# reidprichard/ORC

Measured on AMD Instinct MI355X. Metric: SIMPLE iterations/s (10.24M-cell hex channel equivalents; = iterations/s at N=1), higher is better.
Workload: dtype f64

## Files before the change

### include/orc_amd.h

```cpp
#ifndef ORC_AMD_H
#define ORC_AMD_H

#include <stdint.h>
#include "orc_types.h"

#ifdef __cplusplus
extern "C" {
#endif

typedef struct OrcMesh OrcMesh;
typedef struct OrcSolver OrcSolver;

int orc_init(int device_ordinal);
int orc_device_count(void);
int orc_synchronize(void);
const char *orc_status_string(int status);
const char *orc_last_error(void);
int orc_reload_environment(void);
int orc_device_memory(int64_t *free_bytes, int64_t *total_bytes);
int orc_device_info(char *buf, int cap);
void orc_settings_default(OrcSettings *s);

OrcMesh *orc_mesh_create(int64_t n_cells, int64_t n_faces, int32_t n_zones,
                         const int64_t *face_c0, const int64_t *face_c1, const int32_t *face_zone,
                         const double *face_area, const double *face_normal , const double *face_centroid ,
                         const double *cell_centroid , const double *cell_volume,
                         const int64_t *cell_face_ptr , const int64_t *cell_faces,
                         const int32_t *zone_type, const double *zone_scalar, const double *zone_vector ,
                         int *status);
OrcMesh *orc_mesh_create_reordered(int64_t n_cells, int64_t n_faces, int32_t n_zones,
                                   const int64_t *face_c0, const int64_t *face_c1, const int32_t *face_zone,
                                   const double *face_area, const double *face_normal, const double *face_centroid,
                                   const double *cell_centroid, const double *cell_volume,
                                   const int64_t *cell_face_ptr, const int64_t *cell_faces,
                                   const int32_t *zone_type, const double *zone_scalar, const double *zone_vector,
                                   int32_t ordering, int *status);
int orc_mesh_cell_order(const OrcMesh *m, int64_t *global_ids );
OrcMesh *orc_mesh_create_partitioned(int64_t n_owned, int64_t n_cells, int64_t n_cells_global, int64_t n_faces, int32_t n_zones,
                                     const int64_t *face_c0, const int64_t *face_c1, const int32_t *face_zone, const double *face_area,
                                     const double *face_normal, const double *face_centroid, const double *cell_centroid,
                                     const double *cell_volume, const int64_t *cell_face_ptr, const int64_t *cell_faces,
                                     const int32_t *zone_type, const double *zone_scalar, const double *zone_vector, int32_t n_peers,
                                     const int32_t *peers, const int64_t *send_ptr, const int64_t *send_idx, const int64_t *recv_ptr,
                                     int *status);
int64_t orc_mesh_n_owned(const OrcMesh *m);
typedef struct OrcPartition OrcPartition;
OrcPartition *orc_mesh_partition(int64_t n_cells, int64_t n_faces, const int64_t *face_c0, const int64_t *face_c1, const int32_t *face_zone,
                                 const double *face_area, const double *face_normal, const double *face_centroid,
                                 const double *cell_centroid, const double *cell_volume, const int64_t *cell_face_ptr,
                                 const int64_t *cell_faces, int32_t n_ranks, int32_t rank, int32_t ordering, int *status);
OrcPartition *orc_mesh_partition_owner(int64_t n_cells, int64_t n_faces, const int64_t *face_c0, const int64_t *face_c1, const int32_t *face_zone,
                                       const double *face_area, const double *face_normal, const double *face_centroid,
                                       const double *cell_centroid, const double *cell_volume, const int64_t *cell_face_ptr,
                                       const int64_t *cell_faces, const int32_t *cell_owner, int32_t n_ranks, int32_t rank, int64_t n_global,
                                       int *status);
void orc_partition_destroy(OrcPartition *p);
int orc_partition_sizes(const OrcPartition *p, int64_t *n_owned, int64_t *n_local, int64_t *n_global, int64_t *n_faces, int64_t *n_cell_faces,
                        int32_t *n_peers, int64_t *n_send);
int orc_partition_arrays(const OrcPartition *p, int64_t *face_c0, int64_t *face_c1, int32_t *face_zone, double *face_area, double *face_normal,
                         double *face_centroid, double *cell_centroid, double *cell_volume, int64_t *cell_face_ptr, int64_t *cell_faces,
                         int64_t *global_ids, int64_t *global_face_ids, int32_t *peers, int64_t *send_ptr, int64_t *send_idx, int64_t *recv_ptr);
OrcMesh *orc_partition_upload(const OrcPartition *p, int32_t n_zones, const int32_t *zone_type, const double *zone_scalar,
                              const double *zone_vector, int *status);
int orc_mesh_update_zones(OrcMesh *m, const int32_t *zone_type, const double *zone_scalar, const double *zone_vector);
void orc_mesh_destroy(OrcMesh *m);
int64_t orc_mesh_n_cells(const OrcMesh *m);
int64_t orc_mesh_nnz(const OrcMesh *m);
int orc_mesh_matrix_pattern(const OrcMesh *m, int64_t *row_ptr , int64_t *col_idx );

typedef struct OrcMeshData OrcMeshData;
OrcMeshData *orc_read_mesh(const char *mesh_path, int *status);
void orc_mesh_data_destroy(OrcMeshData *d);
int orc_mesh_data_sizes(const OrcMeshData *d, int32_t *dimensions, int64_t *n_vertices, int64_t *n_cells, int64_t *n_faces,
                        int64_t *n_cell_faces, int64_t *n_face_nodes, int32_t *n_zones);
int orc_mesh_data_arrays(const OrcMeshData *d, int64_t *face_c0, int64_t *face_c1, int32_t *face_zone, double *face_area,
                         double *face_normal, double *face_centroid, double *cell_centroid, double *cell_volume,
                         int64_t *cell_face_ptr, int64_t *cell_faces);
int orc_mesh_data_nodes(const OrcMeshData *d, double *vertices , int64_t *face_node_ptr , int64_t *face_nodes);
int orc_mesh_data_zone(const OrcMeshData *d, int32_t k, uint64_t *zone_id, int32_t *zone_type, double *scalar_value,
                       double *vector_value , char *name, int64_t name_len);
int orc_mesh_data_zone_index(const OrcMeshData *d, const char *name);
int orc_mesh_data_set_zone(OrcMeshData *d, const char *name, int32_t zone_type, double scalar_value, const double *vector_value );
OrcMesh *orc_mesh_upload(const OrcMeshData *d, int *status);
int orc_mesh_sync_zones(OrcMesh *m, const OrcMeshData *d);

int orc_write_data(const char *output_file_name, int64_t n_cells, const double *cell_centroid , const double *u,
                   const double *v, const double *w, const double *p, int decimal_precision);
int orc_read_data(const char *data_file_path, int64_t capacity, double *u, double *v, double *w, double *p, int64_t *n_read);
int orc_write_gradients(const OrcMesh *m, const double *cell_centroid, const double *u, const double *v, const double *w,
                        const double *p, const char *output_file_name, int decimal_precision, const OrcSettings *settings);

int orc_iterative_solve(int64_t n, const int64_t *row_ptr, const int64_t *col_idx, const double *values,
                        const double *b, double *solution_vector , uint64_t iteration_count,
                        int method , double relaxation_factor, double convergence_threshold,
                        int preconditioner );
int orc_iterative_solve3(int64_t n, const int64_t *row_ptr, const int64_t *col_idx, const double *const values[3],
                         const double *const b[3], double *const solution_vectors[3] , uint64_t iteration_count,
                         int method, double relaxation_factor, double convergence_threshold, int preconditioner,
                         int status_out[3]);
int orc_set_breakdown_guard(int on);
int64_t orc_breakdown_guard_events(int reset);
int orc_set_reduction_order(int order);
int64_t orc_last_jacobi_sweeps(void);
int orc_set_gmres_restart(int m);
int orc_last_gmres_stats(int64_t *steps, int64_t *cycles, double *initial_residual, double *final_estimate);
int orc_last_cg_stats(int64_t *iterations, double *initial_residual, double *final_residual, int32_t *event);
int orc_csr_spmv(int64_t n, const int64_t *row_ptr, const int64_t *col_idx, const double *values, const double *x,
                 double *y, int reps, double *avg_ms);

int orc_amg_coarsen(int64_t n, const int64_t *row_ptr, const int64_t *col_idx, const double *values, int64_t *partner ,
                    int64_t *out_n_coarse, int64_t *out_nnz, int64_t *out_row_ptr, int64_t *out_col, double *out_val,
                    int *rounds);

int orc_debug_coloring(int64_t n, const int64_t *row_ptr, const int64_t *col_idx, int32_t *colors , int32_t *n_colors);

int orc_build_momentum_diffusion_matrix(const OrcMesh *m, int diffusion_scheme, double mu,
                                        double *a_values , double *b_u, double *b_v, double *b_w);
int orc_initialize_momentum_matrix(const OrcMesh *m, double *a_values );
int orc_build_momentum_advection_matrices(const OrcMesh *m, double *a_u_values, double *a_v_values, double *a_w_values,
                                          double *b_u, double *b_v, double *b_w, const double *a_di_values,
                                          const double *u, const double *v, const double *w, const double *p,
                                          const OrcSettings *settings, double rho, double peclet[3]);
int orc_build_pressure_correction_matrices(const OrcMesh *m, const double *u, const double *v, const double *w,
                                           const double *p, const double *a_u_values, const double *a_v_values,
                                           const double *a_w_values, const OrcSettings *settings, double rho,
                                           double *a_values , double *b );

int orc_calculate_gradients(const OrcMesh *m, const double *u, const double *v, const double *w, const double *p,
                            const OrcSettings *settings, double *grad_p, double *grad_u);
int orc_check_boundary_conditions(const OrcMesh *m, int *constraint_type);
int orc_initialize_pressure_field(const OrcMesh *m, double *p );
int orc_initialize_flow(const OrcMesh *m, double mu, double rho, uint64_t iteration_count, const OrcSettings *settings,
                        double *u, double *v, double *w, double *p);
int orc_initialize_velocity_field(const OrcMesh *m, const OrcSettings *settings, double *u, double *v, double *w, double *psi);
int orc_initialize_flow_new(const OrcMesh *m, double mu, double rho, uint64_t iteration_count,
                            double *u, double *v, double *w, double *p);
typedef void (*OrcReportFn)(uint64_t iteration, const double mean_velocity[3], const double peclet[3],
                            double velocity_correction, double pressure_correction, double ms_per_iter, void *user);
int orc_solve_steady(OrcMesh *m, double *u, double *v, double *w, double *p, const OrcSettings *settings,
                     double rho, double mu, uint64_t iteration_count, uint64_t reporting_interval,
                     OrcReportFn report_cb, void *user);

OrcSolver *orc_solver_create(OrcMesh *m, const OrcSettings *settings, double rho, double mu, int *status);
void orc_solver_destroy(OrcSolver *s);
int orc_solver_set_fields(OrcSolver *s, const double *u, const double *v, const double *w, const double *p);
int orc_solver_get_fields(OrcSolver *s, double *u, double *v, double *w, double *p);
int orc_solver_iterate(OrcSolver *s, uint64_t iterations, double *report);
int orc_solver_snapshot(OrcSolver *s);
int orc_solver_restore(OrcSolver *s);
int orc_solver_set_pressure_solver(OrcSolver *s, const OrcLinearSolver *c);
int orc_solver_get_pressure_solver(OrcSolver *s, OrcLinearSolver *c, int32_t *enabled);
long long orc_solver_debug_pressure_hierarchies(OrcSolver *s);
int orc_solver_assemble_momentum(OrcSolver *s, double *a_u, double *a_v, double *a_w, double *b_u, double *b_v, double *b_w, double peclet[3]);
int orc_solver_assemble_pressure(OrcSolver *s, double *a_p, double *b_p);

int orc_solver_set_transient(OrcSolver *s, const OrcTransient *t);
int orc_solver_set_time_levels(OrcSolver *s, const double *u_n, const double *v_n, const double *w_n, const double *u_nm1,
                               const double *v_nm1, const double *w_nm1);
int orc_solver_advance(OrcSolver *s, uint64_t time_steps, double *report);
int orc_solve_transient(OrcMesh *m, double *u, double *v, double *w, double *p, const OrcSettings *settings, double rho, double mu,
                        const OrcTransient *t, uint64_t time_steps, uint64_t reporting_interval, OrcReportFn report_cb, void *user);

void orc_scalar_settings_default(OrcScalarSettings *c);
int orc_solver_set_scalar(OrcSolver *s, const OrcScalarSettings *c);
int orc_solver_set_scalar_bc(OrcSolver *s, int32_t zone, int32_t kind, double value);
int orc_solver_set_scalar_field(OrcSolver *s, const double *phi);
int orc_solver_get_scalar_field(OrcSolver *s, double *phi);
int orc_solver_set_scalar_source(OrcSolver *s, const double *source );
int orc_solver_set_scalar_levels(OrcSolver *s, const double *phi_n, const double *phi_nm1 );
int orc_solver_solve_scalar(OrcSolver *s, double report[4]);
int orc_solver_last_scalar_report(OrcSolver *s, double report[4]);
int orc_solver_assemble_scalar(OrcSolver *s, double *a, double *b);
int orc_solver_scalar_boundary_flux(OrcSolver *s, double *per_zone);

int orc_solver_surface_report(OrcSolver *s, const double origin[3], double *per_zone );
int orc_surface_integrals(OrcMesh *m, const double *u, const double *v, const double *w, const double *p,
                          double rho, double mu, const double origin[3], double *per_zone);
int orc_mesh_boundary_index(OrcMesh *m, int64_t *zone_ptr, int32_t *faces, int64_t *n_builds, int32_t *chunk);

int orc_solver_derived_fields(OrcSolver *s, uint32_t mask, double *out );
int orc_derived_fields(OrcMesh *m, const double *u, const double *v, const double *w, const OrcSettings *settings, uint32_t mask,
                       double *out);
int orc_solver_boundary_fields(OrcSolver *s, uint32_t mask, double *out );
int orc_boundary_fields(OrcMesh *m, const double *u, const double *v, const double *w, const double *p, double rho, double mu,
                        uint32_t mask, double *out);
int orc_write_vtu(const char *path, int64_t n_points, const double *points , int64_t n_cells, const int64_t *cell_face_ptr,
                  const int64_t *cell_faces, const int64_t *face_node_ptr, const int64_t *face_nodes, int32_t n_arrays,
                  const char *const *names, const int32_t *components, const double *const *data, int32_t encoding);
int orc_write_vtu_faces(const char *path, int64_t n_points, const double *points, int64_t n_faces, const int64_t *face_ids,
                        const int64_t *face_node_ptr, const int64_t *face_nodes, int32_t n_arrays, const char *const *names,
                        const int32_t *components, const double *const *data, int32_t encoding);

int orc_bench_spmv(OrcSolver *s, int reps, double *avg_ms, double *checksum);
int orc_bench_bicgstab_iteration(OrcSolver *s, int reps, double *avg_ms);
int orc_bench_inloop_products(OrcSolver *s, int reps, double avg_ms[4]);
const char *orc_bench_inloop_variant(void);
int orc_bench_gs_sweep(OrcSolver *s, int reps, double *avg_ms, int *n_colors);
int orc_bench_gs_sweep0(OrcSolver *s, int reps, double avg_ms[2], int *n_colors);
int orc_bench_amg_levels(OrcSolver *s, int reps, int64_t *rows, int64_t *nnz, int64_t *padded, double *avg_ms, int *n_levels);
long long orc_debug_halo_overlaps(void);
int orc_debug_stream_report(char *buf, int cap);
int orc_debug_amg_coarse_product(int64_t n, const int64_t *row_ptr, const int64_t *col_idx, const double *values, int scaled, const double *x,
                                 double *y, int *has_window_mirror);
int orc_debug_amg_packed_mirror(int64_t n, const int64_t *row_ptr, const int64_t *col_idx, const double *values, int64_t sizes[5], int32_t *row_len,
                                int64_t *pk_ptr, int32_t *pk_col, double *pk_val, int64_t *lptr, uint16_t *lidx, int32_t *wcol, int32_t *wsize);
long long orc_debug_collectives(int reset);
int orc_debug_clamp_partials_grid(long long requested);
int orc_debug_max_partials(void);
int orc_debug_amg_certification(long long out[2], int reset);
int orc_debug_amg_setup_stats(long long out[16], int reset);
int orc_debug_xwin_counters(long long out[3], int reset);
long long orc_debug_shared_galerkin(int reset);
enum {
    ORC_PRODUCT_RAGGED = 0,
    ORC_PRODUCT_PACKED = 1,
    ORC_PRODUCT_WINDOW = 2,
    ORC_PRODUCT_GENERIC_SCALED = 3,
    ORC_PRODUCT_WIDE = 4,
    ORC_PRODUCT_NARROW = 5,
    ORC_PRODUCT_NARROW_NT = 6,
    ORC_PRODUCT_MESH = 7,
    ORC_PRODUCT_FAMILIES = 8
};
int orc_debug_product_launches(long long *out, int n_out, int reset);
int orc_profile_enable(int on);
int orc_profile_report(char *buf, int64_t buf_len);

int orc_hex_channel_sizes(int64_t nx, int64_t ny, int64_t nz, int64_t *n_cells, int64_t *n_faces, int64_t *n_cell_faces);
int orc_hex_channel_generate(int64_t nx, int64_t ny, int64_t nz, double lx, double ly, double lz,
                             int64_t *face_c0, int64_t *face_c1, int32_t *face_zone, double *face_area,
                             double *face_normal, double *face_centroid, double *cell_centroid, double *cell_volume,
                             int64_t *cell_face_ptr, int64_t *cell_faces);
int orc_hex_channel_write_msh(const char *path, int64_t nx, int64_t ny, int64_t nz, double lx, double ly, double lz);

int orc_mixed_channel_write_msh(const char *path, int64_t nx, int64_t ny, int64_t nz, double lx, double ly, double lz,
                                int64_t *n_cells, int64_t *n_faces);
int orc_poly_channel_write_msh(const char *path, int64_t nx, int64_t ny, int64_t nz, double lx, double ly, double lz,
                               int64_t *n_cells, int64_t *n_faces);
OrcMeshData *orc_mixed_channel_generate(int64_t nx, int64_t ny, int64_t nz, double lx, double ly, double lz, int polyhedra, int *status);

#define ORC_COMM_ID_BYTES 128
int orc_comm_get_unique_id(unsigned char id[ORC_COMM_ID_BYTES]);
int orc_comm_init(const unsigned char id[ORC_COMM_ID_BYTES], int rank, int world_size);
int orc_comm_finalize(void);
int orc_comm_selftest(void);
int orc_comm_init_self_loop(void);
int orc_comm_set_host_transport(void *exchange_fn, void *allreduce_fn, void *user);

#ifdef __cplusplus
}
#endif
#endif
```

### orc_amd/csrc/amg_hooks.hip

```cpp
#include <algorithm>

#include "amg.hpp"

namespace orc {

static int build_level(const MatView &A, Arena &arena, AmgHierarchy::Level &L) {
    const int64_t n = A.P.n;
    ORC_TRY(arena.alloc((size_t)std::max<int64_t>(n, 1), &L.choice));
    ORC_TRY(arena.alloc((size_t)std::max<int64_t>(n, 1), &L.chooser));
    ORC_TRY(aggregate(A, arena, L.choice, L.chooser, &L.rounds));
    return galerkin(A, arena, L);
}

int amg_debug_coarsen(const MatView &A, Arena &arena, std::vector<int> &choice_h, std::vector<int64_t> &row_ptr_h,
                      std::vector<int64_t> &col_h, std::vector<double> &val_h, int *rounds, const double *x_h, double *y_h, int scaled, int *mirror_out) {
    const int64_t n = A.P.n;
    hipStream_t st = ctx().stream;
    ArenaScope scope(arena);
    AmgHierarchy::Level L;
    ORC_TRY(build_level(A, arena, L));
    if (rounds) *rounds = L.rounds;
    choice_h.resize((size_t)n);
    ORC_HIP(hipMemcpyAsync(choice_h.data(), L.choice, sizeof(int) * (size_t)n, hipMemcpyDeviceToHost, st));
    const int64_t nc = L.n;
    if (mirror_out) *mirror_out = (L.pk.ptr && L.xw.lidx) ? 1 : 0;
    if (x_h && y_h && nc > 0) {
        MatView V = coarse_view(L, A.symmetric);
        double *x, *y, *d1;
        ORC_TRY(arena.alloc((size_t)nc, &x));
        ORC_TRY(arena.alloc((size_t)nc, &y));
        ORC_HIP(hipMemcpyAsync(x, x_h, sizeof(double) * (size_t)nc, hipMemcpyHostToDevice, st));
        if (scaled) {
            ORC_TRY(arena.alloc((size_t)nc, &d1));
            ORC_TRY(diag_inverse_dev(V, d1));
            V.s1 = d1;
            ORC_TRY(materialize_scaled_view(V, 50, arena));
        }
        ORC_TRY(spmv_dev(V, x, y));
        ORC_HIP(hipMemcpyAsync(y_h, y, sizeof(double) * (size_t)nc, hipMemcpyDeviceToHost, st));
        ORC_HIP(hipStreamSynchronize(st));
    }
    std::vector<int> row_len((size_t)nc), col((size_t)std::max<int64_t>(L.padded, 1));
    std::vector<int64_t> slice_ptr((size_t)L.P.n_slices + 1);
    std::vector<double> val((size_t)std::max<int64_t>(L.padded, 1));
    ORC_HIP(hipMemcpyAsync(row_len.data(), L.P.row_len, sizeof(int) * (size_t)nc, hipMemcpyDeviceToHost, st));
    ORC_HIP(hipMemcpyAsync(slice_ptr.data(), L.P.slice_ptr, sizeof(int64_t) * slice_ptr.size(), hipMemcpyDeviceToHost, st));
    ORC_HIP(hipMemcpyAsync(col.data(), L.P.col, sizeof(int) * (size_t)L.padded, hipMemcpyDeviceToHost, st));
    ORC_HIP(hipMemcpyAsync(val.data(), L.val, sizeof(double) * (size_t)L.padded, hipMemcpyDeviceToHost, st));
    ORC_HIP(hipStreamSynchronize(st));
    row_ptr_h.assign((size_t)nc + 1, 0);
    for (int64_t I = 0; I < nc; ++I) row_ptr_h[(size_t)I + 1] = row_ptr_h[(size_t)I] + row_len[(size_t)I];
    col_h.resize((size_t)row_ptr_h[(size_t)nc]);
    val_h.resize((size_t)row_ptr_h[(size_t)nc]);
    for (int64_t I = 0; I < nc; ++I) {
        const int64_t base = slice_ptr[(size_t)(I >> 6)] + (I & 63);
        for (int k = 0; k < row_len[(size_t)I]; ++k) {
            col_h[(size_t)(row_ptr_h[(size_t)I] + k)] = col[(size_t)(base + (int64_t)k * 64)];
            val_h[(size_t)(row_ptr_h[(size_t)I] + k)] = val[(size_t)(base + (int64_t)k * 64)];
        }
    }
    return ORC_OK;
}

int amg_debug_packed(const MatView &A, Arena &arena, int64_t sizes[5], int32_t *row_len_h, int64_t *pk_ptr_h, int32_t *pk_col_h, double *pk_val_h,
                     int64_t *lptr_h, uint16_t *lidx_h, int32_t *wcol_h, int32_t *wsize_h) {
    hipStream_t st = ctx().stream;
    ArenaScope scope(arena);
    AmgHierarchy::Level L;
    ORC_TRY(build_level(A, arena, L));
    const bool mirror = L.pk.ptr && L.xw.lidx;
    const int64_t ns = L.P.n_slices, nb = (ns + 3) / 4;
    sizes[0] = L.n; sizes[1] = ns; sizes[2] = mirror ? L.pk.slots : 0; sizes[3] = 0; sizes[4] = mirror ? nb : 0;
    if (mirror) ORC_HIP(hipMemcpyAsync(&sizes[3], L.xw.lptr + ns, sizeof(int64_t), hipMemcpyDeviceToHost, st));
    ORC_HIP(hipStreamSynchronize(st));
    if (mirror && row_len_h && pk_ptr_h && pk_col_h && pk_val_h && lptr_h && lidx_h && wcol_h && wsize_h) {
        ORC_HIP(hipMemcpyAsync(row_len_h, L.P.row_len, sizeof(int32_t) * (size_t)L.n, hipMemcpyDeviceToHost, st));
        ORC_HIP(hipMemcpyAsync(pk_ptr_h, L.pk.ptr, sizeof(int64_t) * (size_t)(ns + 1), hipMemcpyDeviceToHost, st));
        ORC_HIP(hipMemcpyAsync(pk_col_h, L.pk.col, sizeof(int32_t) * (size_t)sizes[2], hipMemcpyDeviceToHost, st));
        ORC_HIP(hipMemcpyAsync(pk_val_h, L.pk.val, sizeof(double) * (size_t)sizes[2], hipMemcpyDeviceToHost, st));
        ORC_HIP(hipMemcpyAsync(lptr_h, L.xw.lptr, sizeof(int64_t) * (size_t)(ns + 1), hipMemcpyDeviceToHost, st));
        ORC_HIP(hipMemcpyAsync(lidx_h, L.xw.lidx, sizeof(uint16_t) * (size_t)sizes[3], hipMemcpyDeviceToHost, st));
        ORC_HIP(hipMemcpyAsync(wcol_h, L.xw.wcol, sizeof(int32_t) * (size_t)(nb * kXWinCap), hipMemcpyDeviceToHost, st));
        ORC_HIP(hipMemcpyAsync(wsize_h, L.xw.wsize, sizeof(int32_t) * (size_t)nb, hipMemcpyDeviceToHost, st));
        ORC_HIP(hipStreamSynchronize(st));
    }
    return ORC_OK;
}

}
```

### orc_amd/csrc/amg_mirror.hip

```cpp
#include <algorithm>

#include "amg.hpp"

namespace orc {

constexpr int kXBitWords = 8192;
__device__ unsigned long long g_xwin_counters[3];
constexpr int kXBitWordsSmall = 4096;
template <int kWords, bool kSecond>
__global__ __launch_bounds__(kBlock) void xwin_build_k(SellDev P, const int64_t *__restrict__ lptr, int *__restrict__ wcol, int *__restrict__ wsize,
                                                       unsigned short *__restrict__ lidx, int64_t n_blocks, int win_cap, int bit_words, int pass_words,
                                                       int *__restrict__ pending ) {
    if (kSecond && *pending == 0) return;
    __shared__ unsigned bits[kWords];
    __shared__ unsigned short wpre[kWords];
    __shared__ int s_min, s_max, s_part[kBlock];
    const int tid = threadIdx.x, lane = tid & 63, wave = tid >> 6;
    unsigned long long n_built = 0, n_capped = 0, n_spanned = 0;
    for (int64_t b = blockIdx.x; b < n_blocks; b += gridDim.x) {
        if (kSecond && wsize[b] != -2) continue;
        const int64_t row = b * kXWinRows + tid;
        const bool live = row < P.n;
        const int len = live ? P.row_len[row] : 0;
        const int64_t rbase = live ? P.slice_ptr[row >> 6] + (row & 63) : 0;
        if (tid == 0) { s_min = 0x7fffffff; s_max = -1; }
        __syncthreads();
        if (len > 0) {
            atomicMin(&s_min, P.col[rbase]);
            atomicMax(&s_max, P.col[rbase + (int64_t)(len - 1) * 64]);
        }
        __syncthreads();
        const int cmin = s_min, span = s_max - s_min + 1;
        const int words = (span + 31) >> 5;
        if (s_max < 0) {
            if (tid == 0) wsize[b] = 0;
            __syncthreads();
            continue;
        }
        if (!kSecond && words <= bit_words && words > pass_words) {
            if (tid == 0) { wsize[b] = -2; atomicAdd(pending, 1); }
            __syncthreads();
            continue;
        }
        ++n_built;
        if (words > bit_words || words > kWords) {
            if (tid == 0) wsize[b] = -1;
            ++n_spanned;
            __syncthreads();
            continue;
        }
        for (int w = tid; w < words; w += kBlock) bits[w] = 0u;
        __syncthreads();
        for (int k = 0; k < len; ++k) {
            const int c = P.col[rbase + (int64_t)k * 64] - cmin;
            atomicOr(&bits[c >> 5], 1u << (c & 31));
        }
        __syncthreads();
        const int per = (words + kBlock - 1) / kBlock;
        int local = 0;
        for (int w = tid * per; w < words && w < (tid + 1) * per; ++w) local += __popc(bits[w]);
        s_part[tid] = local;
        __syncthreads();
        for (int off = 1; off < kBlock; off <<= 1) {
            const int t = tid >= off ? s_part[tid - off] : 0;
            __syncthreads();
            s_part[tid] += t;
            __syncthreads();
        }
        const int total = s_part[kBlock - 1];
        if (total > win_cap) {
            __syncthreads();
            if (tid == 0) wsize[b] = -1;
            ++n_capped;
            __syncthreads();
            continue;
        }
        int run = s_part[tid] - local;
        int *wc = wcol + b * kXWinCap;
        for (int w = tid * per; w < words && w < (tid + 1) * per; ++w) {
            wpre[w] = (unsigned short)run;
            unsigned m = bits[w];
            while (m) {
                const int bit = __ffs(m) - 1;
                wc[run++] = cmin + (w << 5) + bit;
                m &= m - 1;
            }
        }
        if (tid == 0) wsize[b] = total;
        __syncthreads();
        const int64_t slice = b * 4 + wave;
        if (slice < P.n_slices) {
            const int64_t sbase = P.slice_ptr[slice];
            const int width = (int)((P.slice_ptr[slice + 1] - sbase) >> 6);
            int64_t off = lptr[slice];
            for (int j0 = 0; j0 < width; j0 += kPackChunk) {
                const bool in = j0 < len;
                const unsigned long long m = __ballot(in);
                const int rank = __builtin_amdgcn_mbcnt_hi((unsigned)(m >> 32), __builtin_amdgcn_mbcnt_lo((unsigned)m, 0u));
                if (in) {
                    u32x4_t w = {0u, 0u, 0u, 0u};
#pragma unroll
                    for (int u = 0; u < kPackChunk; ++u) {
                        if (j0 + u < len) {
                            const int c = P.col[sbase + (int64_t)(j0 + u) * 64 + lane] - cmin;
                            const unsigned pos = wpre[c >> 5] + __popc(bits[c >> 5] & ((1u << (c & 31)) - 1u));
                            w[u >> 1] |= pos << (16 * (u & 1));
                        }
                    }
                    *reinterpret_cast<u32x4_t *>(lidx + off + (int64_t)kPackChunk * rank) = w;
                }
                off += (int64_t)kPackChunk * __popcll(m);
            }
        }
        __syncthreads();
    }
    if (tid == 0) {
        if (n_built) atomicAdd(&g_xwin_counters[0], n_built);
        if (n_capped) atomicAdd(&g_xwin_counters[1], n_capped);
        if (n_spanned) atomicAdd(&g_xwin_counters[2], n_spanned);
    }
}

constexpr int kXWinCapSizes = 5;
__device__ __constant__ int kXWinCapSizeDev[kXWinCapSizes] = {2048, 2560, 3200, 4000, kXWinCap};
static const int kXWinCapSize[kXWinCapSizes] = {2048, 2560, 3200, 4000, kXWinCap};
__global__ __launch_bounds__(kBlock) void xwin_cap_k(const int *__restrict__ wsize, int64_t n_blocks, int *__restrict__ over) {
    int c[kXWinCapSizes] = {0, 0, 0, 0, 0};
    for (int64_t b = (int64_t)blockIdx.x * blockDim.x + threadIdx.x; b < n_blocks; b += (int64_t)gridDim.x * blockDim.x) {
        const int ws = wsize[b];
#pragma unroll
        for (int q = 0; q < kXWinCapSizes; ++q) c[q] += ws > kXWinCapSizeDev[q] ? 1 : 0;
    }
#pragma unroll
    for (int q = 0; q < kXWinCapSizes; ++q)
        if (c[q]) atomicAdd(over + q, c[q]);
}

__global__ __launch_bounds__(kBlock) void xwin_stats_k(const int *__restrict__ wcol, const int *__restrict__ wsize, int64_t n_blocks, unsigned long long *__restrict__ out) {
    for (int64_t b = blockIdx.x; b < n_blocks; b += gridDim.x) {
        const int ws = wsize[b];
        if (ws <= 0) { if (threadIdx.x == 0 && ws < 0) atomicAdd(out + 4, 1ull); continue; }
        const int *wc = wcol + b * kXWinCap;
        unsigned long long runs = 0, long_entries = 0;
        for (int j = threadIdx.x; j < ws; j += kBlock) {
            if (j == 0 || wc[j] != wc[j - 1] + 1) {
                ++runs;
                int e = j + 1;
                while (e < ws && wc[e] == wc[e - 1] + 1) ++e;
                if (e - j >= 8) long_entries += (unsigned long long)(e - j);
            }
        }
        atomicAdd(out + 1, runs);
        atomicAdd(out + 2, long_entries);
        if (threadIdx.x == 0) {
            atomicAdd(out + 0, (unsigned long long)ws);
            if (wc[ws - 1] - wc[0] < 65536) atomicAdd(out + 3, 1ull);
        }
    }
}

__global__ __launch_bounds__(64) void narrow_build_k(SellDev P, unsigned short *__restrict__ col16, int *__restrict__ colbase, int *__restrict__ too_wide) {
    const int lane = threadIdx.x;
    for (int64_t slice = blockIdx.x; slice < P.n_slices; slice += gridDim.x) {
        const int64_t row = slice * 64 + lane;
        const int64_t sb = P.slice_ptr[slice];
        const int width = (int)((P.slice_ptr[slice + 1] - sb) >> 6);
        const int len = row < P.n ? P.row_len[row] : 0;
        for (int k = 0; k < width; ++k) {
            const bool in = k < len;
            const int c = in ? P.col[sb + (int64_t)k * 64 + lane] : 0;
            int lo = in ? c : 0x7fffffff, hi = in ? c : -1;
#pragma unroll
            for (int off = 32; off > 0; off >>= 1) {
                lo = min(lo, __shfl_xor(lo, off, 64));
                hi = max(hi, __shfl_xor(hi, off, 64));
            }
            if (hi < 0) lo = 0;
            if (lane == 0) {
                colbase[(sb >> 6) + k] = lo;
                if (hi >= 0 && hi - lo > 65535) atomicOr(too_wide, 1);
            }
            col16[sb + (int64_t)k * 64 + lane] = in ? (unsigned short)(c - lo) : (unsigned short)0;
        }
    }
}

int debug_xwin_counters(long long out[3], bool reset) {
    unsigned long long h[3] = {0, 0, 0};
    ORC_HIP(hipDeviceSynchronize());
    ORC_HIP(hipMemcpyFromSymbol(h, HIP_SYMBOL(g_xwin_counters), sizeof(h)));
    for (int i = 0; i < 3; ++i) out[i] = (long long)h[i];
    if (reset) {
        const unsigned long long z[3] = {0, 0, 0};
        ORC_HIP(hipMemcpyToSymbol(HIP_SYMBOL(g_xwin_counters), z, sizeof(z)));
    }
    return ORC_OK;
}

int narrow_image(SellDev &Pc, Arena &arena, Arena &tmp) {
    const int64_t padded = Pc.padded;
    if (!cfg().spmv_narrow_cols || padded <= 0) return ORC_OK;
    hipStream_t st = ctx().stream;
    unsigned short *c16;
    int *cbase, *wide;
    ORC_TRY(arena.alloc((size_t)padded, &c16));
    ORC_TRY(arena.alloc((size_t)(padded / 64) + 1, &cbase));
    ORC_TRY(tmp.alloc((size_t)1, &wide));
    ORC_HIP(hipMemsetAsync(wide, 0, sizeof(int), st));
    hipLaunchKernelGGL(narrow_build_k, dim3((unsigned)std::max<int64_t>(1, std::min<int64_t>(Pc.n_slices, 256 * 32))), dim3(64), 0, st, Pc, c16, cbase, wide);
    ORC_HIP(hipGetLastError());
    int h_wide = 1;
    ORC_HIP(hipMemcpyAsync(&h_wide, wide, sizeof(int), hipMemcpyDeviceToHost, st));
    ORC_HIP(hipStreamSynchronize(st));
    if (!h_wide) { Pc.col16 = c16; Pc.colbase = cbase; }
    return ORC_OK;
}

int build_windows(const GalerkinSibling *sys, int n_sys, const int64_t *lptr, int64_t pos_slots, Arena &tmp) {
    AmgHierarchy::Level &L = *sys[0].L;
    Arena &arena = *sys[0].arena;
    const SellDev &Pc = L.P;
    const int64_t nc = Pc.n;
    hipStream_t st = ctx().stream;
    const bool trace = cfg().amg_trace;
    const int64_t n_blocks = ((int64_t)Pc.n_slices + 3) / 4;
    int *wcol, *wsize;
    unsigned short *lidx;
    ORC_TRY(arena.alloc((size_t)n_blocks * kXWinCap, &wcol));
    ORC_TRY(arena.alloc((size_t)n_blocks, &wsize));
    ORC_TRY(arena.alloc((size_t)std::max<int64_t>(pos_slots, 1), &lidx));
    const int win_cap = cfg().xwin_cap > 0 ? std::min(kXWinCap, cfg().xwin_cap) : kXWinCap;
    const int bit_words = cfg().xwin_bitwords > 0 ? std::min(kXBitWords, cfg().xwin_bitwords) : kXBitWords;
    const int small_words = cfg().xwin_small_bitwords > 0 ? std::min(kXBitWordsSmall, cfg().xwin_small_bitwords) : kXBitWordsSmall;
    int *pending;
    ORC_TRY(tmp.alloc((size_t)1, &pending));
    ORC_HIP(hipMemsetAsync(pending, 0, sizeof(int), st));
    hipLaunchKernelGGL(HIP_KERNEL_NAME(xwin_build_k<kXBitWordsSmall, false>), dim3((unsigned)std::min<int64_t>(n_blocks, 2048)), dim3(kBlock), 0, st, Pc, lptr, wcol, wsize, lidx,
                       n_blocks, win_cap, bit_words, small_words, pending);
    if (bit_words > small_words)
        hipLaunchKernelGGL(HIP_KERNEL_NAME(xwin_build_k<kXBitWords, true>), dim3((unsigned)std::min<int64_t>(n_blocks, 2048)), dim3(kBlock), 0, st, Pc, lptr, wcol, wsize, lidx,
                           n_blocks, win_cap, bit_words, kXBitWords, pending);
    if (trace) {
        int hp = 0;
        ORC_HIP(hipMemcpyAsync(&hp, pending, sizeof(int), hipMemcpyDeviceToHost, st));
        ORC_HIP(hipStreamSynchronize(st));
        fprintf(stderr, "[amg windows n=%lld] %lld blocks, %d left to the full bitmap\n", (long long)nc, (long long)n_blocks, hp);
    }
    ORC_HIP(hipGetLastError());
    L.xw.wcol = wcol; L.xw.wsize = wsize; L.xw.lidx = lidx; L.xw.lptr = lptr;
    int *over;
    ORC_TRY(tmp.alloc((size_t)kXWinCapSizes, &over));
    ORC_HIP(hipMemsetAsync(over, 0, kXWinCapSizes * sizeof(int), st));
    hipLaunchKernelGGL(xwin_cap_k, dim3((unsigned)std::max<int64_t>(1, std::min<int64_t>((n_blocks + kBlock - 1) / kBlock, 64))), dim3(kBlock), 0, st, (const int *)wsize, n_blocks, over);
    int h_over[kXWinCapSizes];
    ORC_HIP(hipMemcpyAsync(h_over, over, sizeof(h_over), hipMemcpyDeviceToHost, st));
    ORC_HIP(hipStreamSynchronize(st));
    int cap = win_cap;
    for (int q = 0; q < kXWinCapSizes && cfg().xwin_level_cap; ++q)
        if (kXWinCapSize[q] <= win_cap && (int64_t)h_over[q] * 100 <= n_blocks) { cap = kXWinCapSize[q]; break; }
    L.xw.cap = cap;
    if (trace) fprintf(stderr, "[amg windows n=%lld] LDS share %d entries per workgroup (%d of %lld blocks have larger windows)\n", (long long)nc, cap,
                       cap < win_cap ? h_over[std::find(kXWinCapSize, kXWinCapSize + kXWinCapSizes, cap) - kXWinCapSize] : 0, (long long)n_blocks);
    for (int s = 0; s < n_sys; ++s) {
        XWinDev &xw = sys[s].L->xw;
        if (s > 0) xw = L.xw;
        const size_t n_wg = (size_t)((n_blocks + 7) / 8 * 8);
        double *fs;
        unsigned *fc;
        ORC_TRY(sys[s].arena->alloc(2 * n_wg, &fs));
        ORC_TRY(sys[s].arena->alloc((size_t)4, &fc));
        ORC_HIP(hipMemsetAsync(fc, 0, 4 * sizeof(unsigned), st));
        xw.fold_scratch = fs; xw.fold_counter = fc;
    }
    if (cfg().debug_xwin) {
        unsigned long long *d_st, h_st[5];
        ORC_TRY(tmp.alloc((size_t)5, &d_st));
        ORC_HIP(hipMemsetAsync(d_st, 0, sizeof(h_st), st));
        hipLaunchKernelGGL(xwin_stats_k, dim3((unsigned)std::min<int64_t>(n_blocks, 4096)), dim3(kBlock), 0, st, (const int *)wcol, (const int *)wsize, n_blocks, d_st);
        ORC_HIP(hipMemcpyAsync(h_st, d_st, sizeof(h_st), hipMemcpyDeviceToHost, st));
        ORC_HIP(hipStreamSynchronize(st));
        fprintf(stderr, "[orc xwin] rows %lld nnz %lld blocks %lld: window entries %llu (%.1f per row), runs %llu (%.1f entries per run), in runs >= 8: %.1f %%, span < 65536: %llu blocks, no window: %llu\n",
                (long long)nc, (long long)L.pk.total, (long long)n_blocks, h_st[0], (double)h_st[0] / (double)nc, h_st[1], (double)h_st[0] / (double)std::max<unsigned long long>(h_st[1], 1),
                100. * (double)h_st[2] / (double)std::max<unsigned long long>(h_st[0], 1), h_st[3], h_st[4]);
    }
    return ORC_OK;
}

}
```

### orc_amd/csrc/api_linalg.cpp

```cpp
#include <algorithm>

#include "linalg.hpp"

namespace orc {
static SolveStats g_last_stats;
SolveStats &last_stats() { return g_last_stats; }

struct UserMatrix {
    SellMatrix pat;
    DevBuf<double> csr_vals, vals;
    MatView view;
    int load(int64_t n, const int64_t *row_ptr, const int64_t *col_idx, const double *values) {
        ORC_TRY(sell_from_csr_host(n, n, row_ptr, col_idx, pat));
        ORC_TRY(csr_vals.upload(values, (size_t)pat.nnz));
        ORC_TRY(vals.alloc((size_t)std::max<int64_t>(pat.padded, 1)));
        ORC_TRY(sell_import_values(pat, csr_vals.p, vals.p));
        view.P = pat.dev();
        view.val = vals.p;
        view.symmetric = pat.symmetric;
        return ORC_OK;
    }
};
}

extern "C" {

int orc_iterative_solve(int64_t n, const int64_t *row_ptr, const int64_t *col_idx, const double *values, const double *b,
                        double *solution_vector, uint64_t iteration_count, int method, double relaxation_factor,
                        double convergence_threshold, int preconditioner) {
    using namespace orc;
    ORC_TRY(ensure_init());
    if (n < 0 || !row_ptr || (!col_idx && n > 0) || (!values && n > 0) || !b || !solution_vector)
        return set_error(ORC_ERR_BAD_ARGUMENT, "null argument");
    UserMatrix m;
    ORC_TRY(m.load(n, row_ptr, col_idx, values));
    const size_t nn = (size_t)std::max<int64_t>(n, 1);
    DevBuf<double> db, dx;
    ORC_TRY(db.alloc(nn));
    ORC_TRY(dx.alloc(nn));
    ORC_TRY(db.upload(b, (size_t)n));
    ORC_TRY(dx.upload(solution_vector, (size_t)n));
    Arena arena;
    g_last_stats = SolveStats();
    int st = iterative_solve_dev(m.view, db.p, dx.p, iteration_count, method, relaxation_factor, convergence_threshold, preconditioner,
                                 arena, &g_last_stats);
    int st2 = dx.download(solution_vector, (size_t)n);
    return st != ORC_OK ? st : st2;
}

int orc_iterative_solve3(int64_t n, const int64_t *row_ptr, const int64_t *col_idx, const double *const values[3], const double *const b[3],
                         double *const solution_vectors[3], uint64_t iteration_count, int method, double relaxation_factor,
                         double convergence_threshold, int preconditioner, int status_out[3]) {
    using namespace orc;
    ORC_TRY(ensure_init());
    if (n < 0 || !row_ptr || (!col_idx && n > 0) || !values || !b || !solution_vectors) return set_error(ORC_ERR_BAD_ARGUMENT, "null argument");
    if (method != ORC_SOLVER_BICGSTAB && method != ORC_SOLVER_MULTIGRID)
        return set_error(ORC_ERR_BAD_ARGUMENT, "orc_iterative_solve3: BiCGSTAB and Multigrid arms only (method %d)", method);
    SellMatrix pat;
    ORC_TRY(sell_from_csr_host(n, n, row_ptr, col_idx, pat));
    const size_t nn = (size_t)std::max<int64_t>(n, 1);
    DevBuf<double> csr_vals, vals[3], db[3], dx[3];
    MatView3 A3;
    A3.P = pat.dev();
    for (int k = 0; k < 3; ++k) {
        ORC_TRY(csr_vals.upload(values[k], (size_t)pat.nnz));
        ORC_TRY(vals[k].alloc((size_t)std::max<int64_t>(pat.padded, 1)));
        ORC_TRY(sell_import_values(pat, csr_vals.p, vals[k].p));
        ORC_HIP(hipStreamSynchronize(ctx().stream));
        ORC_TRY(db[k].alloc(nn));
        ORC_TRY(dx[k].alloc(nn));
        ORC_TRY(db[k].upload(b[k], (size_t)n));
        ORC_TRY(dx[k].upload(solution_vectors[k], (size_t)n));
        A3.val[k] = vals[k].p;
    }
    Arena arena;
    int st = ORC_OK;
    int st3[3] = {ORC_OK, ORC_OK, ORC_OK};
    if (!triple_supported()) {
        for (int k = 0; k < 3; ++k) {
            MatView A;
            A.P = pat.dev();
            A.val = vals[k].p;
            A.symmetric = pat.symmetric;
            SolveStats stats;
            st3[k] = iterative_solve_dev(A, db[k].p, dx[k].p, iteration_count, method, relaxation_factor, convergence_threshold, preconditioner, arena, &stats);
            if (st == ORC_OK && st3[k] != ORC_OK && st3[k] != ORC_ERR_MULTIGRID_DIVERGED) st = st3[k];
        }
    } else if (method == ORC_SOLVER_BICGSTAB) {
        double *b3, *x3;
        ORC_TRY(arena.alloc(3 * nn, &b3));
        ORC_TRY(arena.alloc(3 * nn, &x3));
        ORC_TRY(interleave3_dev(db[0].p, db[1].p, db[2].p, b3, n));
        ORC_TRY(interleave3_dev(dx[0].p, dx[1].p, dx[2].p, x3, n));
        st = bicgstab3_dev(A3, b3, x3, iteration_count, preconditioner, arena);
        if (st == ORC_OK) st = deinterleave3_dev(x3, dx[0].p, dx[1].p, dx[2].p, n);
    } else {
        TripleLane lanes[3];
        Arena hier[3], vec[3], scratch[3];
        SiblingPairing sibling;
        hipStream_t streams[6] = {nullptr, nullptr, nullptr, nullptr, nullptr, nullptr};
        for (int k = 0; k < 6 && st == ORC_OK; ++k)
            st = stream_create(&streams[k], kPlainStream, k, "solve3");
        for (int k = 0; k < 3; ++k) {
            lanes[k].setup_stream = streams[2 * k]; lanes[k].solve_stream = streams[2 * k + 1];
            lanes[k].hier_arena = &hier[k]; lanes[k].vec_arena = &vec[k]; lanes[k].scratch_arena = &scratch[k];
            lanes[k].symmetric = pat.symmetric;
        }
        const double *bb[3] = {db[0].p, db[1].p, db[2].p};
        double *xx[3] = {dx[0].p, dx[1].p, dx[2].p};
        if (st == ORC_OK)
            st = multigrid_arm3_dev(A3, bb, xx, iteration_count, relaxation_factor, convergence_threshold, preconditioner, arena, lanes, &sibling, st3);
        (void)hipDeviceSynchronize();
        for (int k = 0; k < 6; ++k)
            if (streams[k]) stream_destroy(streams[k]);
    }
    for (int k = 0; k < 3; ++k) {
        const int st2 = dx[k].download(solution_vectors[k], (size_t)n);
        if (st == ORC_OK) st = st2;
        if (status_out) status_out[k] = st3[k];
    }
    if (!status_out && st == ORC_OK)
        for (int k = 0; k < 3 && st == ORC_OK; ++k) st = st3[k];
    return st;
}

int orc_csr_spmv(int64_t n, const int64_t *row_ptr, const int64_t *col_idx, const double *values, const double *x, double *y,
                 int reps, double *avg_ms) {
    using namespace orc;
    ORC_TRY(ensure_init());
    if (n < 0 || !row_ptr || !x || !y) return set_error(ORC_ERR_BAD_ARGUMENT, "null argument");
    SellMatrix pat;
    ORC_TRY(sell_from_csr_host(n, n, row_ptr, col_idx, pat));
    const size_t nn = (size_t)std::max<int64_t>(n, 1);
    DevBuf<double> csr_vals, vals, dx, dy;
    ORC_TRY(csr_vals.upload(values, (size_t)pat.nnz));
    ORC_TRY(vals.alloc((size_t)std::max<int64_t>(pat.padded, 1)));
    ORC_TRY(sell_import_values(pat, csr_vals.p, vals.p));
    ORC_TRY(dx.alloc(nn));
    ORC_TRY(dy.alloc(nn));
    ORC_TRY(dx.upload(x, (size_t)n));
    MatView A;
    A.P = pat.dev();
    A.val = vals.p;
    if (reps < 1) reps = 1;
    hipEvent_t e0, e1;
    ORC_HIP(hipEventCreate(&e0));
    ORC_HIP(hipEventCreate(&e1));
    ORC_TRY(spmv_dev(A, dx.p, dy.p));
    ORC_HIP(hipEventRecord(e0, ctx().stream));
    for (int i = 1; i < reps; ++i) ORC_TRY(spmv_dev(A, dx.p, dy.p));
    ORC_HIP(hipEventRecord(e1, ctx().stream));
    ORC_HIP(hipEventSynchronize(e1));
    float ms = 0.f;
    ORC_HIP(hipEventElapsedTime(&ms, e0, e1));
    if (avg_ms) *avg_ms = reps > 1 ? (double)ms / (reps - 1) : 0.;
    (void)hipEventDestroy(e0);
    (void)hipEventDestroy(e1);
    return dy.download(y, (size_t)n);
}

int orc_amg_coarsen(int64_t n, const int64_t *row_ptr, const int64_t *col_idx, const double *values, int64_t *partner,
                    int64_t *out_n_coarse, int64_t *out_nnz, int64_t *out_row_ptr, int64_t *out_col, double *out_val, int *rounds) {
    using namespace orc;
    ORC_TRY(ensure_init());
    UserMatrix m;
    ORC_TRY(m.load(n, row_ptr, col_idx, values));
    Arena arena;
    std::vector<int> choice;
    std::vector<int64_t> rp, ci;
    std::vector<double> v;
    ORC_TRY(amg_debug_coarsen(m.view, arena, choice, rp, ci, v, rounds));
    if (partner) for (int64_t i = 0; i < n; ++i) partner[i] = choice[(size_t)i];
    if (out_n_coarse) *out_n_coarse = (int64_t)rp.size() - 1;
    if (out_nnz) *out_nnz = (int64_t)ci.size();
    if (out_col) {
        std::copy(rp.begin(), rp.end(), out_row_ptr);
        std::copy(ci.begin(), ci.end(), out_col);
        std::copy(v.begin(), v.end(), out_val);
    }
    return ORC_OK;
}

int orc_debug_amg_coarse_product(int64_t n, const int64_t *row_ptr, const int64_t *col_idx, const double *values, int scaled, const double *x,
                                 double *y, int *has_window_mirror) {
    using namespace orc;
    ORC_TRY(ensure_init());
    if (n < 1 || !row_ptr || !col_idx || !values || !x || !y) return set_error(ORC_ERR_BAD_ARGUMENT, "null argument");
    UserMatrix m;
    ORC_TRY(m.load(n, row_ptr, col_idx, values));
    Arena arena;
    std::vector<int> choice;
    std::vector<int64_t> rp, ci;
    std::vector<double> v;
    return amg_debug_coarsen(m.view, arena, choice, rp, ci, v, nullptr, x, y, scaled, has_window_mirror);
}

int orc_debug_amg_packed_mirror(int64_t n, const int64_t *row_ptr, const int64_t *col_idx, const double *values, int64_t sizes[5], int32_t *row_len,
                                int64_t *pk_ptr, int32_t *pk_col, double *pk_val, int64_t *lptr, uint16_t *lidx, int32_t *wcol, int32_t *wsize) {
    using namespace orc;
    ORC_TRY(ensure_init());
    if (n < 1 || !row_ptr || !col_idx || !values || !sizes) return set_error(ORC_ERR_BAD_ARGUMENT, "null argument");
    UserMatrix m;
    ORC_TRY(m.load(n, row_ptr, col_idx, values));
    Arena arena;
    return amg_debug_packed(m.view, arena, sizes, row_len, pk_ptr, pk_col, pk_val, lptr, lidx, wcol, wsize);
}

int orc_debug_coloring(int64_t n, const int64_t *row_ptr, const int64_t *col_idx, int32_t *colors, int32_t *n_colors) {
    using namespace orc;
    ORC_TRY(ensure_init());
    SellMatrix pat;
    ORC_TRY(sell_from_csr_host(n, n, row_ptr, col_idx, pat));
    std::vector<int> c;
    int nc = 0;
    ORC_TRY(gs_debug_coloring(pat.dev(), c, &nc));
    for (int64_t i = 0; i < n; ++i) colors[i] = c[(size_t)i];
    if (n_colors) *n_colors = nc;
    return ORC_OK;
}

int64_t orc_last_jacobi_sweeps(void) { return orc::g_last_stats.jacobi_sweeps; }

int orc_set_gmres_restart(int m) {
    orc::ctx().gmres_restart = m;
    return ORC_OK;
}

int orc_last_gmres_stats(int64_t *steps, int64_t *cycles, double *initial_residual, double *final_estimate) {
    const orc::SolveStats &s = orc::g_last_stats;
    if (steps) *steps = s.gmres_steps;
    if (cycles) *cycles = s.gmres_cycles;
    if (initial_residual) *initial_residual = s.gmres_beta0;
    if (final_estimate) *final_estimate = s.gmres_estimate;
    return ORC_OK;
}

int orc_last_cg_stats(int64_t *iterations, double *initial_residual, double *final_residual, int32_t *event) {
    const orc::SolveStats &s = orc::g_last_stats;
    if (iterations) *iterations = s.cg_iterations;
    if (initial_residual) *initial_residual = s.cg_beta0;
    if (final_residual) *final_residual = s.cg_residual;
    if (event) *event = s.cg_event;
    return ORC_OK;
}

}
```

### orc_amd/csrc/arms.hpp

```cpp
#pragma once
#include <vector>

namespace orc {

inline bool reference_order(const MatView &A) { return ctx().reduction_order == ORC_REDUCTION_REFERENCE && A.halo == nullptr; }

int reduce_partials(const double *partials, int count, int nq, double *out, bool global = false);

int spmv_grid(int32_t n_slices);
int product_store(const MatView &A, const double *x, double *y, const double *skip_flags);
int product_store_sum(const MatView &A, const double *x, double *y, double *partials, int *grid_out, const double *skip_flags);
int product_residual(const MatView &A, const double *x, const double *b, double *r, double *p, double *partials, int *grid_out, const double *skip_flags);
int product_residual_norm(const MatView &A, const double *x, const double *b, double *r, double *partials, int *grid_out, const double *skip_flags);
int product_ts(const MatView &A, const double *s, double *t, double *partials, int *grid_out, const double *skip_flags);
int product_store_dot(const MatView &A, const double *p, double *q, double *partials, int *grid_out, const double *skip_flags);
int product_store_sum3(const MatView3 &A, const double *x3, double *y3, double *partials, int *grid_out);
int product_residual3(const MatView3 &A, const double *x3, const double *b3, double *r3, double *p3, double *partials, int *grid_out);
int product_ts3(const MatView3 &A, const double *s3, double *t3, double *partials, int *grid_out);

int jacobi_dev(const MatView &A, const double *b, double *x, uint64_t iteration_count, double relaxation_factor, double threshold, Arena &arena,
               SolveStats *stats, int *status_out);
int bicgstab_dev(const MatView &A, const double *b, double *x, uint64_t iteration_count, Arena &arena);
int multigrid_arm_dev(const MatView &A, const double *b, double *x, uint64_t iteration_count, double relaxation_factor,
                      double convergence_threshold, int preconditioner, Arena &arena, SolveStats *stats, int smoother);
int gs_arm_dev(const MatView &A, const double *b, double *x, uint64_t iteration_count, double relaxation_factor, int method, Arena &arena);
int gmres_dev(const MatView &A, const double *b, double *x, uint64_t iteration_count, double convergence_threshold, Arena &arena,
              SolveStats *stats);
int cg_dev(const MatView &A, const double *b, double *x, uint64_t iteration_count, double convergence_threshold, int preconditioner, Arena &arena,
           SolveStats *stats);
SolveStats &last_stats();

int debug_product_launches(long long *out, int n_out, bool reset);
void debug_amg_certification(long long out[2], bool reset);
void debug_amg_setup_stats(long long out[16], bool reset);
long long debug_shared_galerkin(bool reset);
int debug_xwin_counters(long long out[3], bool reset);
int amg_debug_coarsen(const MatView &A, Arena &arena, std::vector<int> &choice_h, std::vector<int64_t> &row_ptr_h,
                      std::vector<int64_t> &col_h, std::vector<double> &val_h, int *rounds, const double *x_h = nullptr, double *y_h = nullptr,
                      int scaled = 0, int *mirror_out = nullptr);
int amg_debug_packed(const MatView &A, Arena &arena, int64_t sizes[5], int32_t *row_len_h, int64_t *pk_ptr_h, int32_t *pk_col_h, double *pk_val_h,
                     int64_t *lptr_h, uint16_t *lidx_h, int32_t *wcol_h, int32_t *wsize_h);
void gs_forget_pattern(const void *col_ptr);
int bench_gs_sweep_dev(const MatView &A, const double *b, double *x, int reps, Arena &arena, float *ms_per_sweep, int *n_colors);
int bench_gs_sweep0_dev(const MatView A[3], const double *const b[3], int reps, Arena &arena, float ms[2], int *n_colors);
int gs_debug_coloring(const SellDev &P, std::vector<int> &colors, int *n_colors);

}
```

### orc_amd/csrc/config.hpp

```cpp
#pragma once
#include <string>

namespace orc {

struct Config {
    bool triple_momentum = true;
    bool concurrent_momentum = true;
    bool two_stream_multigrid = true;
    bool early_p_hierarchy = true;
    int stream_priorities = 3;
    bool halo_overlap = true;
    bool amg_da = true;
    int amg_da_steps = 1 << 22;
    int amg_da_group = 0;
    bool amg_sibling = true;
    bool amg_shared_scaling = true;
    bool amg_shared_galerkin = true;
    bool amg_l0_mirror = true;
    std::string galerkin_groups;
    int spmv_nt = -1;
    bool spmv_narrow_cols = true;
    int materialize_scaling = 4;
    int spmv_xwin_min_nnz = 24;
    int spmv_grid = 0;
    int xwin_wgs_per_cu = 8;
    int xwin_cap = 0;
    int xwin_bitwords = 0;
    int xwin_small_bitwords = 0;
    bool xwin_wg_per_block = true;
    bool xwin_level_cap = true;
    bool gs_slotspace = true;
    bool trace = false;
    bool amg_trace = false;
    bool arena_trace = false;
    bool debug_nan = false;
    bool debug_xwin = false;
    int debug_sync = 0;
    std::string inject_lane_error;
    bool keep_priority_classes = false;
};

const Config &cfg();
void config_reload();

}
```

### orc_amd/csrc/linalg.hpp

```cpp
#pragma once
#include <condition_variable>
#include <functional>
#include <mutex>
#include "common.hpp"
#include "halo.hpp"

namespace orc {

struct SellDev {
    int64_t n = 0;
    int64_t ncols = 0;
    int32_t n_slices = 0;
    int32_t ragged = 0;
    int64_t padded = 0;
    const int64_t *slice_ptr = nullptr;
    const int32_t *row_len = nullptr;
    const int32_t *col = nullptr;
    const int32_t *diag_pos = nullptr;
    const uint16_t *col16 = nullptr;
    const int32_t *colbase = nullptr;
    const long long *rows_base = nullptr;
    const int32_t *rows_intra = nullptr;
    const int32_t *rows_col = nullptr;
    const int64_t *csr_row_ptr = nullptr;
    int64_t nnz = 0;
};

constexpr int kPackChunk = 8;
struct PackedDev {
    const int64_t *ptr = nullptr;
    const int32_t *col = nullptr;
    const double *val = nullptr;
    int64_t total = 0;
    int64_t slots = 0;
};

constexpr int kXWinRows = 256;
constexpr int kXWinCap = 5000;
struct XWinDev {
    const int32_t *wcol = nullptr;
    const int32_t *wsize = nullptr;
    const uint16_t *lidx = nullptr;
    const int64_t *lptr = nullptr;
    int32_t cap = kXWinCap;
    double *fold_scratch = nullptr;
    unsigned *fold_counter = nullptr;
};

struct RowsDev {
    const long long *slice_base = nullptr;
    const int32_t *intra_off = nullptr;
    const int32_t *col = nullptr;
    const double *val = nullptr;
};

struct MatView {
    SellDev P;
    const double *val = nullptr;
    const double *s1 = nullptr;
    const double *s2 = nullptr;
    int nt = 0;
    PackedDev pk;
    XWinDev xw;
    RowsDev rows;
    bool symmetric = true;
    bool persistent_pattern = false;
    HaloPlan *halo = nullptr;
    int32_t slice_lo = 0, slice_hi = -1, part_stride = 0, part_base = 0;
};

struct MatView3 {
    SellDev P;
    const double *val[3] = {nullptr, nullptr, nullptr};
    const double *s1 = nullptr, *s2 = nullptr;
    bool mesh_pattern = false;
    int nt = 0;
    HaloPlan *halo = nullptr;
    int32_t slice_lo = 0, slice_hi = -1, part_stride = 0, part_base = 0;
};

struct SellMatrix {
    int64_t n = 0, ncols = 0, nnz = 0, padded = 0;
    int32_t n_slices = 0;
    bool symmetric = true;
    int ragged = 0;
    DevBuf<int64_t> slice_ptr;
    DevBuf<int32_t> row_len, col, diag_pos, colbase;
    DevBuf<uint16_t> col16;
    DevBuf<int64_t> csr_row_ptr;
    DevBuf<long long> rows_base;
    DevBuf<int32_t> rows_intra, rows_col;
    SellDev dev() const {
        SellDev d;
        d.n = n; d.ncols = ncols; d.n_slices = n_slices; d.ragged = ragged; d.padded = padded; d.slice_ptr = slice_ptr.p; d.row_len = row_len.p; d.col = col.p; d.diag_pos = diag_pos.p;
        d.col16 = col16.p; d.colbase = colbase.p;
        d.rows_base = rows_base.p; d.rows_intra = rows_intra.p; d.rows_col = rows_col.p; d.csr_row_ptr = csr_row_ptr.p; d.nnz = nnz;
        return d;
    }
};

int sell_from_csr_host(int64_t n, int64_t ncols, const int64_t *row_ptr, const int64_t *col, SellMatrix &out);
int sell_import_values(const SellMatrix &m, const double *csr_vals_dev, double *sell_vals_dev);
int sell_export_values(const SellMatrix &m, const double *sell_vals_dev, double *csr_vals_dev);
int sell_rows_values_dev(const SellDev &P, const double *sell_vals_dev, double *rows_vals_dev);

struct SolveSide {
    hipStream_t stream = nullptr;
    Arena *arena = nullptr;
    hipEvent_t ev_setup = nullptr, ev_solve = nullptr;
};

struct AmgHierarchy {
    struct Level {
        int *choice = nullptr, *chooser = nullptr;
        SellDev P;
        double *val = nullptr;
        PackedDev pk;
        XWinDev xw;
        RowsDev rows;
        bool rows_transient = false;
        int64_t n = 0, padded = 0;
        int rounds = 0;
    } level[4];
    int n_levels = 0;
    int64_t n_fine = 0;
};
inline MatView coarse_view(const AmgHierarchy::Level &L, bool symmetric) {
    MatView V;
    V.P = L.P; V.val = L.val; V.pk = L.pk; V.xw = L.xw; V.rows = L.rows; V.symmetric = symmetric;
    return V;
}

struct SiblingPairing {
    static constexpr int kLevels = 8;
    DevBuf<int> buf[kLevels];
    int64_t n[kLevels] = {0};
    hipEvent_t ready[kLevels] = {nullptr};
    bool published[kLevels] = {false};
    bool leader_done = true;
    std::mutex mu;
    std::condition_variable cv;
    ~SiblingPairing();
    void begin(bool leader_will_run);
    int publish(int level, const int *choice, int64_t rows, hipStream_t stream);
    const int *wait(int level, int64_t rows, hipStream_t stream);
    void finish();

    struct Offer {
        bool made = false, ok = false;
        const MatView *view = nullptr;
        Arena *arena = nullptr, *rows_arena = nullptr;
        hipEvent_t view_ready = nullptr;
        bool answered = false, adopted = false;
        AmgHierarchy::Level *level = nullptr;
    } offer[2];
    int expected_offers = 0;
    hipEvent_t ops_ready = nullptr;
    const int *lead_choice = nullptr, *lead_chooser = nullptr;
    void set_expected(int n);
    int make_offer(int slot, const MatView *view, Arena *arena, Arena *rows_arena, AmgHierarchy::Level *level, hipStream_t stream);
    void withdraw(int slot);
    bool wait_answer(int slot, hipStream_t stream);
    int collect_offers(Offer *out[2]);
    int answer(const bool adopted[2], const int *choice, const int *chooser, hipStream_t stream);
};

struct SolveStats {
    SiblingPairing *sibling = nullptr;
    int sibling_role = 0;
    SolveSide *side = nullptr;
    const AmgHierarchy *hierarchy = nullptr;
    int64_t jacobi_sweeps = 0;
    int64_t gmres_steps = 0, gmres_cycles = 0;
    double gmres_beta0 = 0., gmres_estimate = 0.;
    int64_t cg_iterations = 0;
    double cg_beta0 = 0., cg_residual = 0.;
    int cg_event = 0;
    int amg_levels = 0;
    int64_t amg_rows[8] = {0};
    int64_t amg_nnz[8] = {0};
    int amg_rounds[8] = {0};
};

int iterative_solve_dev(const MatView &A, const double *b, double *x, uint64_t iteration_count, int method,
                        double relaxation_factor, double convergence_threshold, int preconditioner, Arena &arena,
                        SolveStats *stats);

int multigrid_prepare_dev(const MatView &A, int preconditioner, Arena &arena, AmgHierarchy &H, SiblingPairing *sibling = nullptr,
                          int sibling_role = 0, Arena *scratch = nullptr);
int diag_inverse_dev(const MatView &A, double *dinv);
int scale_vec_dev(const double *s, const double *b, double *out, int64_t n);
int multigrid_coarse_part_dev(const MatView &A, const double *r, double *x, uint64_t iteration_count, double relaxation_factor,
                              double convergence_threshold, int preconditioner, Arena &arena, SolveStats *stats, int *dev_status);

int spmv_dev(const MatView &A, const double *x, double *y);
int bench_bicgstab_dev(const MatView &A, const double *b, double *x, int reps, Arena &arena, float *ms);

int residual_dev(const MatView &A, const double *b, const double *x, double *r);
int residual_norm2_dev(const MatView &A, const double *b, const double *x, double *partials, double *out, double *r_scratch = nullptr);
int dot_reference(const double *a, const double *b, int64_t n, double *out, const double *skip_flags);
int sum_reference(const double *a, int64_t n, double *out);

int interleave3_dev(const double *a, const double *b, const double *c, double *out3, int64_t n);
int deinterleave3_dev(const double *in3, double *a, double *b, double *c, int64_t n);
int diag_inverse3_dev(const MatView3 &A, double *dinv3);
int spmv3_dev(const MatView3 &A, const double *x3, double *y3);
int residual3_dev(const MatView3 &A, const double *b3, double *x3, double *r3);
int residual_norm2_3_dev(const MatView3 &A, const double *b3, double *x3, double *partials , double *out3);
int bicgstab3_dev(const MatView3 &A, const double *b3, double *x3, uint64_t iteration_count, int preconditioner, Arena &arena);
int bench_inloop_products_dev(const MatView &A, const double *x, double *y, double *partials, int reps, float ms[2]);
int bench_inloop_products3_dev(const MatView3 &A, const double *x3, double *y3, double *partials, int reps, float ms[2]);
int matview_stream_nt(const MatView &A);
int materialize_scaled_view(MatView &A, uint64_t iteration_count, Arena &arena);
int materialize_scaled_view3(MatView3 &A, uint64_t iteration_count, Arena &arena);
struct ScaledOperator {
    MatView A;
    const double *dinv = nullptr;
    uint64_t iterations = 0;
};
struct ScaledOperator3 {
    MatView3 A;
    const double *dinv3 = nullptr;
    uint64_t iterations = 0;
};
int jacobi_scaling_prepare_dev(const MatView &A, uint64_t iteration_count, Arena &arena, ScaledOperator &S);
int jacobi_scaling_prepare3_dev(const MatView3 &A, uint64_t iteration_count, Arena &arena, ScaledOperator3 &S);
int bicgstab_scaled_dev(const ScaledOperator &S, const double *b, double *x, Arena &arena);
int bicgstab3_scaled_dev(const ScaledOperator3 &S, const double *b3, double *x3, Arena &arena);
bool triple_supported();

struct TripleLane {
    hipStream_t setup_stream = nullptr, solve_stream = nullptr;
    Arena *hier_arena = nullptr, *vec_arena = nullptr;
    Arena *scratch_arena = nullptr;
    AmgHierarchy hierarchy;
    SolveStats stats;
    bool symmetric = true;
};
int multigrid_arm3_dev(const MatView3 &A3, const double *const b[3], double *const x[3], uint64_t iteration_count, double relaxation_factor,
                       double convergence_threshold, int preconditioner, Arena &arena, TripleLane lanes[3], SiblingPairing *sibling, int status_out[3],
                       const std::function<void()> &on_hierarchies_built = nullptr);

int gs_bicgstab3_dev(const MatView A[3], const double *const b[3], double *const x[3], uint64_t iteration_count, Arena &arena);
bool gs_slot_space_enabled();

int vec_fill(double *x, double v, int64_t n);
int vec_copy(double *dst, const double *src, int64_t n);

}

#include "arms.hpp"
```

### orc_amd/csrc/linalg_kernels.hpp

```cpp
#pragma once
#include "linalg.hpp"

namespace orc {

__device__ __forceinline__ double view_value(const MatView &A, int64_t row, int64_t pos) {
    double v = A.val[pos];
    if (A.s1) v = A.s1[row] * v;
    if (A.s2) v = A.s2[row] * v;
    return v;
}

template <bool NT, class T>
__device__ __forceinline__ T ld_stream(const T *p) {
    if (NT) return __builtin_nontemporal_load(p);
    return *p;
}

typedef unsigned u32x4_t __attribute__((ext_vector_type(4)));
typedef int i32x2_t __attribute__((ext_vector_type(2)));
typedef double f64x2_t __attribute__((ext_vector_type(2)));

__device__ __forceinline__ int packed_pair(bool in, int &off) {
    const unsigned long long m = __ballot(in);
    const int rank = __builtin_amdgcn_mbcnt_hi((unsigned)(m >> 32), __builtin_amdgcn_mbcnt_lo((unsigned)m, 0u));
    const int p = in ? off + rank : (m != 0ull ? off : off - 1);
    off += __popcll(m);
    return p;
}

__device__ __forceinline__ double fold_partials_block(const double *__restrict__ partials, int count, double *lds16 ) {
    const int lane = threadIdx.x & 63, w = threadIdx.x >> 6;
    double a[4], b[4];
#pragma unroll
    for (int p = 0; p < 4; ++p) {
        const int vt = (w + 4 * p) * 64 + lane;
        a[p] = vt < count ? partials[vt] : 0.;
        b[p] = vt + 1024 < count ? partials[vt + 1024] : 0.;
    }
    __syncthreads();
#pragma unroll
    for (int p = 0; p < 4; ++p) {
        const int vt = (w + 4 * p) * 64 + lane;
        double v = 0.;
        if (vt < count) v += a[p];
        if (vt + 1024 < count) v += b[p];
        v = wave_sum(v);
        if (lane == 0) lds16[w + 4 * p] = v;
    }
    __syncthreads();
    double r = 0.;
#pragma unroll
    for (int i = 0; i < 16; ++i) r += lds16[i];
    return r;
}

template <int NQ>
__device__ __forceinline__ void fold_partials_multi(const double *__restrict__ partials, int count, double *lds , double (&out)[NQ]) {
    const int lane = threadIdx.x & 63, w = threadIdx.x >> 6;
    double a[NQ][4], b[NQ][4];
#pragma unroll
    for (int q = 0; q < NQ; ++q) {
#pragma unroll
        for (int p = 0; p < 4; ++p) {
            const int vt = (w + 4 * p) * 64 + lane;
            a[q][p] = vt < count ? partials[(size_t)q * count + vt] : 0.;
            b[q][p] = vt + 1024 < count ? partials[(size_t)q * count + vt + 1024] : 0.;
        }
    }
    __syncthreads();
#pragma unroll
    for (int q = 0; q < NQ; ++q) {
#pragma unroll
        for (int p = 0; p < 4; ++p) {
            const int vt = (w + 4 * p) * 64 + lane;
            double v = 0.;
            if (vt < count) v += a[q][p];
            if (vt + 1024 < count) v += b[q][p];
            v = wave_sum(v);
            if (lane == 0) lds[q * 16 + w + 4 * p] = v;
        }
    }
    __syncthreads();
#pragma unroll
    for (int q = 0; q < NQ; ++q) {
        double r = 0.;
#pragma unroll
        for (int i = 0; i < 16; ++i) r += lds[q * 16 + i];
        out[q] = r;
    }
}

struct SliceWalk {
    int64_t begin, end, step;
    __device__ __forceinline__ SliceWalk(int32_t n_slices, int32_t first = 0) : SliceWalk(n_slices, first, (int)blockIdx.x, (int)gridDim.x) {}
    __device__ __forceinline__ SliceWalk(int32_t n_slices, int32_t first, int block, int grid) {
        const int waves = blockDim.x >> 6;
        const int wave = __builtin_amdgcn_readfirstlane((int)(threadIdx.x >> 6));
        if ((grid & 7) == 0 && grid >= 8) {
            const int xcd = block & 7, bl = block >> 3, nb = grid >> 3;
            const int64_t spx = ((int64_t)(n_slices - first) + 7) / 8;
            const int64_t lo = (int64_t)first + (int64_t)xcd * spx;
            int64_t hi = lo + spx;
            if (hi > n_slices) hi = n_slices;
            begin = lo + (int64_t)bl * waves + wave;
            end = hi;
            step = (int64_t)nb * waves;
        } else {
            begin = (int64_t)first + (int64_t)block * waves + wave;
            end = n_slices;
            step = (int64_t)grid * waves;
        }
    }
};

enum { kSpmvPlain = 0, kSpmvRagged = 1, kSpmvPacked = 2 };
template <class Epi, int kLayout = kSpmvPlain, bool kNoGather = false, bool kGuard = false>
__global__ __launch_bounds__(kBlock) void spmv_k(MatView A, const double *__restrict__ x, Epi epi, double *__restrict__ partials,
                                                 const double *__restrict__ skip_flags ) {
    __shared__ double lds[8];
    if (skip_flags && (skip_flags[0] != 0. || skip_flags[1] != 0.)) return;
    const int lane = threadIdx.x & 63;
    double r0 = 0., r1 = 0.;
    SliceWalk w(A.P.n_slices);
    for (int64_t slice = w.begin; slice < w.end; slice += w.step) {
        const int64_t row = slice * 64 + lane;
        const int64_t base = A.P.slice_ptr[slice];
        const int width = (int)((A.P.slice_ptr[slice + 1] - base) >> 6);
        const bool live = row < A.P.n;
        const int len = live ? A.P.row_len[row] : 0;
        const double s1 = (A.s1 && live) ? A.s1[row] : 1.;
        const double s2 = (A.s2 && live) ? A.s2[row] : 1.;
        double acc = 0.;
        const i32x2_t *pk_c = kLayout == kSpmvPacked ? reinterpret_cast<const i32x2_t *>(A.pk.col + A.pk.ptr[slice]) : nullptr;
        const f64x2_t *pk_v = kLayout == kSpmvPacked ? reinterpret_cast<const f64x2_t *>(A.pk.val + A.pk.ptr[slice]) : nullptr;
        int pk_off = 0;
        const int last = (kLayout == kSpmvRagged ? (len > 0 ? len : 1) : width) - 1;
        const int lane_c = live ? lane : (int)((A.P.n - 1) & 63);
        for (int k0 = 0; k0 < width; k0 += 8) {
            int c[8];
            double v[8], xv[8];
            if (kLayout == kSpmvPacked) {
#pragma unroll
                for (int q = 0; q < 4; ++q) {
                    const int p = packed_pair(k0 + 2 * q < len, pk_off);
                    const i32x2_t cc = pk_c[p];
                    const f64x2_t vv = pk_v[p];
                    c[2 * q] = cc.x; c[2 * q + 1] = cc.y;
                    v[2 * q] = vv.x; v[2 * q + 1] = vv.y;
                }
            } else {
#pragma unroll
                for (int u = 0; u < 8; ++u) {
                    if (kGuard) {
                        if (k0 + u < width) {
                            const int kk = kLayout == kSpmvPlain ? k0 + u : (k0 + u < last ? k0 + u : last);
                            const int64_t p = kLayout == kSpmvPlain ? (base + (int64_t)k0 * 64 + lane_c) + (int64_t)u * 64 : base + (int64_t)kk * 64 + lane_c;
                            c[u] = A.P.col[p];
                            v[u] = A.val[p];
                        } else { c[u] = 0; v[u] = 0.; }
                    } else {
                        const int kk = k0 + u < last ? k0 + u : last;
                        const int64_t p = base + (int64_t)kk * 64 + lane_c;
                        c[u] = A.P.col[p];
                        v[u] = A.val[p];
                    }
                }
            }
#pragma unroll
            for (int u = 0; u < 8; ++u) {
                if (kGuard) { if (k0 + u < width) xv[u] = x[c[u]]; else xv[u] = 0.; }
                else xv[u] = x[kNoGather ? (int)(live ? row : 0) + (c[u] & 0) : c[u]];
            }
#pragma unroll
            for (int u = 0; u < 8; ++u) {
                double t = v[u];
                if (A.s1) t = s1 * t;
                if (A.s2) t = s2 * t;
                const double next = acc + t * xv[u];
                acc = (k0 + u < len) ? next : acc;
            }
        }
        if (live) epi.apply(row, acc, r0, r1);
    }
    if (Epi::kReductions > 0) {
        double t = block_sum(r0, lds);
        if (threadIdx.x == 0) partials[blockIdx.x] = t;
    }
    if (Epi::kReductions > 1) {
        double t = block_sum(r1, lds);
        if (threadIdx.x == 0) partials[gridDim.x + blockIdx.x] = t;
    }
}

template <class Epi, bool kRagged = false, bool kMesh = false, bool kNarrow = false, bool kScaled = true, bool kNT = false>
__global__ __launch_bounds__(kBlock) void spmv_uniform_k(MatView A, const double *__restrict__ x, Epi epi, double *__restrict__ partials,
                                                 const double *__restrict__ skip_flags ) {
    __shared__ double lds[8];
    if (skip_flags && (skip_flags[0] != 0. || skip_flags[1] != 0.)) return;
    const int lane = threadIdx.x & 63;
    double r0 = 0., r1 = 0.;
    SliceWalk w(A.slice_hi >= 0 ? A.slice_hi : A.P.n_slices, A.slice_lo);
    for (int64_t slice = w.begin; slice < w.end; slice += w.step) {
        const int64_t row = slice * 64 + lane;
        const int64_t base = A.P.slice_ptr[slice];
        const int width = (int)((A.P.slice_ptr[slice + 1] - base) >> 6);
        const bool live = row < A.P.n;
        const int len = live ? A.P.row_len[row] : 0;
        const double s1 = (kScaled && A.s1 && live) ? A.s1[row] : 1.;
        const double s2 = (kScaled && A.s2 && live) ? A.s2[row] : 1.;
        double acc = 0.;
        const int32_t *__restrict__ cb = kNarrow ? A.P.colbase + (base >> 6) : nullptr;
        for (int k0 = 0; k0 < width; k0 += 8) {
            int c[8];
            double v[8], xv[8];
            const int64_t p0 = base + (int64_t)k0 * 64 + lane;
            if (kNarrow) {
#pragma unroll
                for (int u = 0; u < 8; ++u) {
                    const bool in = k0 + u < width;
                    c[u] = in ? cb[k0 + u] + (int)ld_stream<kNT>(A.P.col16 + p0 + (int64_t)u * 64) : 0;
                    v[u] = in ? ld_stream<kNT>(A.val + p0 + (int64_t)u * 64) : 0.;
                }
            } else {
#pragma unroll
                for (int u = 0; u < 8; ++u) {
                    const bool in = k0 + u < (kRagged ? len : width);
                    c[u] = in ? ld_stream<kNT>(A.P.col + p0 + (int64_t)u * 64) : 0;
                    v[u] = in ? ld_stream<kNT>(A.val + p0 + (int64_t)u * 64) : 0.;
                }
            }
#pragma unroll
            for (int u = 0; u < 8; ++u) xv[u] = (k0 + u < len) ? x[c[u]] : 0.;
#pragma unroll
            for (int u = 0; u < 8; ++u) {
                if (k0 + u < len) {
                    double t = v[u];
                    if (kScaled && A.s1) t = s1 * t;
                    if (kScaled && A.s2) t = s2 * t;
                    acc += t * xv[u];
                }
            }
        }
        if (live) epi.apply(row, acc, r0, r1);
    }
    const int pstride = A.part_stride > 0 ? A.part_stride : (int)gridDim.x;
    if (Epi::kReductions > 0) {
        double t = block_sum(r0, lds);
        if (threadIdx.x == 0) partials[A.part_base + blockIdx.x] = t;
    }
    if (Epi::kReductions > 1) {
        double t = block_sum(r1, lds);
        if (threadIdx.x == 0) partials[pstride + A.part_base + blockIdx.x] = t;
    }
}


struct __attribute__((aligned(8))) Vec3d { double a, b, c; };

template <class Epi3, int kChunk = 4, bool kMesh = false, bool kNarrow = false, bool kScaled = true, bool kNT = false>
__global__ __launch_bounds__(kBlock) void spmv3_uniform_k(MatView3 A, const double *__restrict__ x3, Epi3 epi, double *__restrict__ partials) {
    __shared__ double lds[8];
    const int lane = threadIdx.x & 63;
    const Vec3d *__restrict__ xv3 = reinterpret_cast<const Vec3d *>(x3);
    const Vec3d *__restrict__ s1v = reinterpret_cast<const Vec3d *>(A.s1);
    const Vec3d *__restrict__ s2v = reinterpret_cast<const Vec3d *>(A.s2);
    const int vgrid = (int)gridDim.x;
    for (int vb = blockIdx.x; vb < vgrid; vb += gridDim.x) {
    double red[3][2] = {{0., 0.}, {0., 0.}, {0., 0.}};
    SliceWalk w(A.slice_hi >= 0 ? A.slice_hi : A.P.n_slices, A.slice_lo, vb, vgrid);
    for (int64_t slice = w.begin; slice < w.end; slice += w.step) {
        const int64_t row = slice * 64 + lane;
        const int64_t base = A.P.slice_ptr[slice];
        const int width = (int)((A.P.slice_ptr[slice + 1] - base) >> 6);
        const bool live = row < A.P.n;
        const int len = live ? A.P.row_len[row] : 0;
        Vec3d s1 = {1., 1., 1.}, s2 = {1., 1., 1.};
        if (kScaled && A.s1 && live) s1 = s1v[row];
        if (kScaled && A.s2 && live) s2 = s2v[row];
        double acc0 = 0., acc1 = 0., acc2 = 0.;
        const int32_t *__restrict__ cb = kNarrow ? A.P.colbase + (base >> 6) : nullptr;
        for (int k0 = 0; k0 < width; k0 += kChunk) {
            int c[kChunk];
            double v0[kChunk], v1[kChunk], v2[kChunk];
            Vec3d xv[kChunk];
            const int64_t p0 = base + (int64_t)k0 * 64 + lane;
#pragma unroll
            for (int u = 0; u < kChunk; ++u) {
                const bool in = k0 + u < width;
                if (kNarrow) c[u] = in ? cb[k0 + u] + (int)ld_stream<kNT>(A.P.col16 + p0 + (int64_t)u * 64) : 0;
                else c[u] = in ? ld_stream<kNT>(A.P.col + p0 + (int64_t)u * 64) : 0;
                v0[u] = in ? ld_stream<kNT>(A.val[0] + p0 + (int64_t)u * 64) : 0.;
                v1[u] = in ? ld_stream<kNT>(A.val[1] + p0 + (int64_t)u * 64) : 0.;
                v2[u] = in ? ld_stream<kNT>(A.val[2] + p0 + (int64_t)u * 64) : 0.;
            }
#pragma unroll
            for (int u = 0; u < kChunk; ++u) {
                if (k0 + u < len) xv[u] = xv3[c[u]];
                else xv[u] = Vec3d{0., 0., 0.};
            }
#pragma unroll
            for (int u = 0; u < kChunk; ++u) {
                if (k0 + u < len) {
                    double t0 = v0[u], t1 = v1[u], t2 = v2[u];
                    if (kScaled && A.s1) { t0 = s1.a * t0; t1 = s1.b * t1; t2 = s1.c * t2; }
                    if (kScaled && A.s2) { t0 = s2.a * t0; t1 = s2.b * t1; t2 = s2.c * t2; }
                    acc0 += t0 * xv[u].a;
                    acc1 += t1 * xv[u].b;
                    acc2 += t2 * xv[u].c;
                }
            }
        }
        if (live) {
            const double acc[3] = {acc0, acc1, acc2};
            epi.apply(row, acc, red);
        }
    }
#pragma unroll
    for (int s = 0; s < 3; ++s) {
#pragma unroll
        for (int q = 0; q < Epi3::kReductions; ++q) {
            const double t = block_sum(red[s][q], lds);
            if (threadIdx.x == 0) partials[(size_t)(s * Epi3::kReductions + q) * (A.part_stride > 0 ? A.part_stride : vgrid) + A.part_base + vb] = t;
        }
    }
    }
}

template <class Epi, bool kScaled = true, bool kNT = false>
__global__ __launch_bounds__(kBlock) void spmv_xwin_k(MatView A, const double *__restrict__ x, Epi epi, double *__restrict__ partials,
                                                      const double *__restrict__ skip_flags) {
    __shared__ double lds[8];
    extern __shared__ __align__(16) double xs[];
    constexpr int kC = kPackChunk;
    if (skip_flags && (skip_flags[0] != 0. || skip_flags[1] != 0.)) return;
    const int lane = threadIdx.x & 63, wave = __builtin_amdgcn_readfirstlane((int)(threadIdx.x >> 6));
    double r0 = 0., r1 = 0.;
    const int64_t n_blocks = ((int64_t)A.P.n_slices + 3) >> 2;
    int64_t b_begin, b_end, b_step;
    if ((gridDim.x & 7) == 0 && gridDim.x >= 8) {
        const int xcd = blockIdx.x & 7, bl = blockIdx.x >> 3, nb = gridDim.x >> 3;
        const int64_t per = (n_blocks + 7) / 8;
        b_begin = (int64_t)xcd * per + bl;
        b_end = (int64_t)(xcd + 1) * per < n_blocks ? (int64_t)(xcd + 1) * per : n_blocks;
        b_step = nb;
    } else {
        b_begin = blockIdx.x; b_end = n_blocks; b_step = gridDim.x;
    }
    for (int64_t b = b_begin; b < b_end; b += b_step) {
        const int ws_built = A.xw.wsize[b];
        const int ws = ws_built <= A.xw.cap ? ws_built : -1;
        const int64_t slice = b * 4 + wave;
        const bool has_slice = slice < A.P.n_slices;
        const int64_t row = slice * 64 + lane;
        const bool live = has_slice && row < A.P.n;
        int width = 0, len = 0;
        int64_t pk_off = 0, lp_off = 0;
        if (has_slice) {
            const int64_t base = A.P.slice_ptr[slice];
            width = (int)((A.P.slice_ptr[slice + 1] - base) >> 6);
            len = live ? A.P.row_len[row] : 0;
            pk_off = A.pk.ptr[slice];
            lp_off = ws >= 0 ? A.xw.lptr[slice] : 0;
        }
        const int64_t sb = __builtin_amdgcn_readfirstlane((int)(pk_off & 0xffffffff)) | ((int64_t)__builtin_amdgcn_readfirstlane((int)(pk_off >> 32)) << 32);
        const int64_t lb = __builtin_amdgcn_readfirstlane((int)(lp_off & 0xffffffff)) | ((int64_t)__builtin_amdgcn_readfirstlane((int)(lp_off >> 32)) << 32);
        const u32x4_t *s_pos = reinterpret_cast<const u32x4_t *>(A.xw.lidx + lb);
        const f64x2_t *s_val = reinterpret_cast<const f64x2_t *>(A.pk.val + sb);
        int poff = 0, voff = 0;
        u32x4_t c, cn;
        f64x2_t v[kC / 2], vn[kC / 2];
        auto issue = [&](int k0, u32x4_t &cc, f64x2_t (&vv)[kC / 2]) {
            {
                const unsigned long long m = __ballot(k0 < len);
                const int rank = __builtin_amdgcn_mbcnt_hi((unsigned)(m >> 32), __builtin_amdgcn_mbcnt_lo((unsigned)m, 0u));
                cc = ld_stream<kNT>(s_pos + poff + (k0 < len ? rank : 0));
                poff += __popcll(m);
            }
#pragma unroll
            for (int q = 0; q < kC / 2; ++q) vv[q] = ld_stream<kNT>(s_val + packed_pair(k0 + 2 * q < len, voff));
        };
        if (ws > 0) {
            const int32_t *wc = A.xw.wcol + b * kXWinCap;
            for (int j0 = 0; j0 < ws; j0 += 8 * kBlock) {
                int wj[8];
                double xw[8];
#pragma unroll
                for (int q = 0; q < 8; ++q) {
                    const int j = j0 + q * kBlock + (int)threadIdx.x;
                    wj[q] = ld_stream<kNT>(wc + (j < ws ? j : 0));
                }
#pragma unroll
                for (int q = 0; q < 8; ++q) xw[q] = x[wj[q]];
#pragma unroll
                for (int q = 0; q < 8; ++q) {
                    const int j = j0 + q * kBlock + (int)threadIdx.x;
                    if (j < ws) xs[j] = xw[q];
                }
            }
        }
        __syncthreads();
        if (has_slice) {
            const double s1 = (kScaled && A.s1 && live) ? A.s1[row] : 1.;
            const double s2 = (kScaled && A.s2 && live) ? A.s2[row] : 1.;
            double acc = 0.;
            if (ws >= 0) {
                auto consume = [&](int k0, const u32x4_t &cc, const f64x2_t (&vv)[kC / 2]) {
                    double xv[kC];
#pragma unroll
                    for (int q = 0; q < kC / 2; ++q) {
                        const unsigned w = cc[q];
                        xv[2 * q] = xs[w & 0xffffu];
                        xv[2 * q + 1] = xs[w >> 16];
                    }
#pragma unroll
                    for (int u = 0; u < kC; ++u) {
                        double t = vv[u >> 1][u & 1];
                        if (kScaled && A.s1) t = s1 * t;
                        if (kScaled && A.s2) t = s2 * t;
                        const double next = acc + t * xv[u];
                        acc = (k0 + u < len) ? next : acc;
                    }
                };
                if (width > 0) issue(0, c, v);
                int k0 = 0;
                for (; k0 + kC < width; k0 += 2 * kC) {
                    issue(k0 + kC, cn, vn);
                    consume(k0, c, v);
                    if (k0 + 2 * kC < width) issue(k0 + 2 * kC, c, v);
                    consume(k0 + kC, cn, vn);
                }
                if (k0 < width) consume(k0, c, v);
            } else {
                const i32x2_t *s_col = reinterpret_cast<const i32x2_t *>(A.pk.col + sb);
                for (int k0 = 0; k0 < width; k0 += 8) {
                    int cg[8];
                    double vg[8], xv[8];
#pragma unroll
                    for (int q = 0; q < 4; ++q) {
                        const int p = packed_pair(k0 + 2 * q < len, voff);
                        const i32x2_t cc = ld_stream<kNT>(s_col + p);
                        const f64x2_t vv = ld_stream<kNT>(s_val + p);
                        cg[2 * q] = cc.x; cg[2 * q + 1] = cc.y;
                        vg[2 * q] = vv.x; vg[2 * q + 1] = vv.y;
                    }
#pragma unroll
                    for (int u = 0; u < 8; ++u) xv[u] = x[cg[u]];
#pragma unroll
                    for (int u = 0; u < 8; ++u) {
                        double t = vg[u];
                        if (kScaled && A.s1) t = s1 * t;
                        if (kScaled && A.s2) t = s2 * t;
                        const double next = acc + t * xv[u];
                        acc = (k0 + u < len) ? next : acc;
                    }
                }
            }
            if (live) epi.apply(row, acc, r0, r1);
        }
        __syncthreads();
    }
    if (Epi::kReductions > 0 && A.xw.fold_scratch) {
        __shared__ int s_last;
        const int nwg = (int)gridDim.x;
        const double t0 = block_sum(r0, lds);
        const double t1 = Epi::kReductions > 1 ? block_sum(r1, lds) : 0.;
        if (threadIdx.x == 0) {
            __hip_atomic_store(A.xw.fold_scratch + blockIdx.x, t0, __ATOMIC_RELAXED, __HIP_MEMORY_SCOPE_AGENT);
            if (Epi::kReductions > 1) __hip_atomic_store(A.xw.fold_scratch + nwg + blockIdx.x, t1, __ATOMIC_RELAXED, __HIP_MEMORY_SCOPE_AGENT);
            __builtin_amdgcn_s_waitcnt(0);
            s_last = __hip_atomic_fetch_add(A.xw.fold_counter, 1u, __ATOMIC_RELAXED, __HIP_MEMORY_SCOPE_AGENT) == (unsigned)(nwg - 1);
        }
        __syncthreads();
        if (s_last) {
            const double *fs = A.xw.fold_scratch;
#pragma unroll
            for (int q = 0; q < Epi::kReductions; ++q) {
                double v = 0.;
                for (int i0 = threadIdx.x; i0 < nwg; i0 += 8 * kBlock) {
                    double t[8];
#pragma unroll
                    for (int u = 0; u < 8; ++u) {
                        const int i = i0 + u * kBlock;
                        t[u] = i < nwg ? __hip_atomic_load(fs + (size_t)q * nwg + i, __ATOMIC_RELAXED, __HIP_MEMORY_SCOPE_AGENT) : 0.;
                    }
#pragma unroll
                    for (int u = 0; u < 8; ++u) v += t[u];
                }
                v = block_sum(v, lds);
                if (threadIdx.x == 0) partials[q] = v;
            }
            if (threadIdx.x == 0) __hip_atomic_store(A.xw.fold_counter, 0u, __ATOMIC_RELAXED, __HIP_MEMORY_SCOPE_AGENT);
        }
        return;
    }
    if (Epi::kReductions > 0) {
        double t = block_sum(r0, lds);
        if (threadIdx.x == 0) partials[blockIdx.x] = t;
    }
    if (Epi::kReductions > 1) {
        double t = block_sum(r1, lds);
        if (threadIdx.x == 0) partials[gridDim.x + blockIdx.x] = t;
    }
}

}
```

### orc_amd/csrc/runtime.cpp

```cpp
#include <algorithm>
#include <cstdarg>
#include <mutex>

#include "config.hpp"
#include "linalg.hpp"

namespace orc {

static thread_local Ctx *t_ctx_override = nullptr;

Ctx &ctx() {
    static Ctx c;
    return t_ctx_override ? *t_ctx_override : c;
}

CtxScope::CtxScope(Ctx *local) { t_ctx_override = local; }
CtxScope::~CtxScope() { t_ctx_override = nullptr; }

int set_error(int code, const char *fmt, ...) {
    char buf[1024];
    va_list ap;
    va_start(ap, fmt);
    vsnprintf(buf, sizeof(buf), fmt, ap);
    va_end(ap);
    ctx().last_error = buf;
    return code;
}


static Config g_cfg;
static std::mutex g_cfg_mu;
static bool g_cfg_loaded = false;
static int env_int(const char *name, int dflt) { const char *e = getenv(name); return (e && *e) ? atoi(e) : dflt; }
static bool env_on(const char *name, bool dflt) { const char *e = getenv(name); return (e && *e) ? atoi(e) != 0 : dflt; }
static bool env_set(const char *name) { return getenv(name) != nullptr; }
static std::string env_str(const char *name) { const char *e = getenv(name); return e ? std::string(e) : std::string(); }

void config_reload() {
    Config c;
    c.triple_momentum = env_on("ORC_TRIPLE_MOMENTUM", true);
    c.concurrent_momentum = env_on("ORC_CONCURRENT_MOMENTUM", true);
    c.two_stream_multigrid = env_on("ORC_TWO_STREAM_MULTIGRID", true);
    c.early_p_hierarchy = env_on("ORC_EARLY_P_HIERARCHY", true);
    c.stream_priorities = env_int("ORC_STREAM_PRIORITIES", 3);
    c.halo_overlap = env_on("ORC_HALO_OVERLAP", true);
    c.amg_da = env_on("ORC_AMG_DA", true);
    c.amg_da_steps = std::max(1, env_int("ORC_AMG_DA_STEPS", 1 << 22));
    c.amg_da_group = env_int("ORC_AMG_DA_GROUP", 0);
    c.amg_sibling = env_on("ORC_AMG_SIBLING", true);
    c.amg_shared_scaling = env_on("ORC_AMG_SHARED_SCALING", true);
    c.amg_shared_galerkin = env_on("ORC_AMG_SHARED_GALERKIN", true);
    c.amg_l0_mirror = env_on("ORC_AMG_L0_MIRROR", true);
    c.galerkin_groups = env_str("ORC_GALERKIN_GROUPS");
    c.spmv_nt = env_int("ORC_SPMV_NT", -1);
    c.spmv_narrow_cols = env_on("ORC_SPMV_NARROW_COLS", true);
    c.materialize_scaling = env_int("ORC_MATERIALIZE_SCALING", 4);
    c.spmv_xwin_min_nnz = env_int("ORC_SPMV_XWIN_MIN_NNZ", 24);
    c.spmv_grid = env_int("ORC_SPMV_GRID", 0);
    c.xwin_wgs_per_cu = std::max(1, env_int("ORC_XWIN_WGS_PER_CU", 8));
    c.xwin_cap = env_int("ORC_XWIN_CAP", 0);
    c.xwin_bitwords = env_int("ORC_XWIN_BITWORDS", 0);
    c.xwin_small_bitwords = env_int("ORC_XWIN_SMALL_BITWORDS", 0);
    c.xwin_wg_per_block = env_on("ORC_XWIN_WG_PER_BLOCK", true);
    c.xwin_level_cap = env_on("ORC_XWIN_LEVEL_CAP", true);
    c.gs_slotspace = env_on("ORC_GS_SLOTSPACE", true);
    c.trace = env_set("ORC_DEBUG_TRACE");
    c.amg_trace = env_set("ORC_AMG_TRACE");
    c.arena_trace = env_set("ORC_ARENA_TRACE");
    c.debug_nan = env_set("ORC_DEBUG_NAN");
    c.debug_xwin = env_set("ORC_DEBUG_XWIN") || env_on("ORC_XWIN_STATS", false);
    c.debug_sync = env_int("ORC_DEBUG_SYNC", 0);
    c.inject_lane_error = env_str("ORC_DEBUG_INJECT_LANE_ERROR");
    c.keep_priority_classes = env_on("ORC_DEBUG_KEEP_PRIORITY_CLASSES", false);
    std::lock_guard<std::mutex> lk(g_cfg_mu);
    g_cfg = c;
    g_cfg_loaded = true;
}

const Config &cfg() {
    if (!g_cfg_loaded) config_reload();
    return g_cfg;
}

struct StreamEntry { hipStream_t st; std::string name; int priority; int role; };
static std::mutex g_streams_mu;
static std::vector<StreamEntry> g_streams;

static void stream_register(hipStream_t st, const char *name, int priority, int role) {
    std::lock_guard<std::mutex> lk(g_streams_mu);
    g_streams.push_back(StreamEntry{st, name ? name : "?", priority, role});
}

int stream_role(hipStream_t st) {
    std::lock_guard<std::mutex> lk(g_streams_mu);
    for (const auto &e : g_streams)
        if (e.st == st) return e.role;
    return kPlainStream;
}

int stream_create(hipStream_t *out, int role, int lane, const char *name) {
    const int prio_mode = (role == kPlainStream || (device_shared_between_ranks() && !cfg().keep_priority_classes)) ? 0 : cfg().stream_priorities;
    int least = 0, greatest = 0, prio = 0;
    bool with_prio = false;
    if (prio_mode != 0 && hipDeviceGetStreamPriorityRange(&least, &greatest) == hipSuccess && least != greatest) {
        int klass = prio_mode == 1 ? lane : (role == kSolveStream ? 2 : 0);
        if (prio_mode == 3) klass = role == kSolveStream ? 0 : 2;
        prio = klass == 0 ? greatest : (klass == 2 ? least : (least + greatest) / 2);
        with_prio = true;
    }
    if (with_prio) ORC_HIP(hipStreamCreateWithPriority(out, hipStreamNonBlocking, prio));
    else ORC_HIP(hipStreamCreateWithFlags(out, hipStreamNonBlocking));
    char full[96];
    snprintf(full, sizeof(full), "%s[%d]", name ? name : "stream", lane);
    stream_register(*out, full, with_prio ? prio : 0, role);
    return ORC_OK;
}

void stream_destroy(hipStream_t st) {
    if (!st) return;
    {
        std::lock_guard<std::mutex> lk(g_streams_mu);
        for (size_t i = 0; i < g_streams.size(); ++i)
            if (g_streams[i].st == st) { g_streams.erase(g_streams.begin() + (long)i); break; }
    }
    (void)hipStreamDestroy(st);
}

int ensure_init() {
    if (ctx().inited) return ORC_OK;
    return orc_init(-1);
}

Arena::~Arena() {
    if (cfg().arena_trace && !chunks_.empty())
        fprintf(stderr, "[orc arena %p] %zu chunk(s), reserved %.2f GB, high water %.2f GB\n", (void *)this, chunks_.size(), (double)reserved() / 1e9, (double)high_ / 1e9);
    for (auto &c : chunks_)
        if (c.p) (void)hipFree(c.p);
}

int Arena::reset() {
    cur_ = 0;
    off_ = 0;
    live_ = 0;
    peak_ = std::max(peak_, high_);
    const size_t used = peak_;
    high_ = 0;
    if (chunks_.empty() || used == 0) return ORC_OK;
    if (chunks_.size() == 1) return ORC_OK;
    const size_t want = used + used / 16 + ((size_t)16 << 20);
    if (cfg().arena_trace) fprintf(stderr, "[orc arena %p] compacting %zu chunk(s), reserved %.2f GB -> %.2f GB\n", (void *)this, chunks_.size(), (double)reserved() / 1e9, (double)want / 1e9);
    for (auto &c : chunks_)
        if (c.p) (void)hipFree(c.p);
    chunks_.clear();
    Chunk c{nullptr, want};
    hipError_t e = hipMalloc((void **)&c.p, want);
    if (e != hipSuccess) return set_error(ORC_ERR_HIP, "arena hipMalloc(%zu) failed: %s", want, hipGetErrorString(e));
    chunks_.push_back(c);
    return ORC_OK;
}

size_t Arena::reserved() const {
    size_t t = 0;
    for (auto &c : chunks_) t += c.size;
    return t;
}

int Arena::alloc_bytes(size_t bytes, void **out) {
    bytes = (bytes + 255) & ~(size_t)255;
    if (bytes == 0) bytes = 256;
    while (true) {
        if (cur_ < chunks_.size()) {
            Chunk &c = chunks_[cur_];
            if (off_ + bytes <= c.size) {
                *out = c.p + off_;
                off_ += bytes;
                live_ += bytes;
                if (live_ > high_) high_ = live_;
                return ORC_OK;
            }
            ++cur_;
            off_ = 0;
            continue;
        }
        size_t want = std::max<size_t>(bytes, (size_t)64 << 20);
        want = std::max(want, reserved() / 2);
        Chunk c{nullptr, want};
        hipError_t e = hipMalloc((void **)&c.p, want);
        if (e != hipSuccess) return set_error(ORC_ERR_HIP, "arena hipMalloc(%zu) failed: %s", want, hipGetErrorString(e));
        chunks_.push_back(c);
    }
}

}

extern "C" {

int orc_device_count(void) {
    int n = 0;
    if (hipGetDeviceCount(&n) != hipSuccess) return 0;
    return n;
}

int orc_init(int device_ordinal) {
    orc::Ctx &c = orc::ctx();
    int n = orc_device_count();
    if (n <= 0) return orc::set_error(ORC_ERR_NO_DEVICE, "no HIP device visible: liborc_amd has no CPU fallback");
    if (!c.inited) orc::config_reload();
    if (c.inited && (device_ordinal < 0 || device_ordinal == c.device)) return ORC_OK;
    if (device_ordinal < 0) device_ordinal = 0;
    if (device_ordinal >= n) return orc::set_error(ORC_ERR_BAD_ARGUMENT, "device %d out of range (%d visible)", device_ordinal, n);
    ORC_HIP(hipSetDevice(device_ordinal));
    if (c.stream) { orc::stream_destroy(c.stream); c.stream = nullptr; }
    ORC_TRY(orc::stream_create(&c.stream, orc::kSolveStream, 0, "library"));
    c.device = device_ordinal;
    if (c.guard_events) { (void)hipFree(c.guard_events); c.guard_events = nullptr; }
    ORC_HIP(hipMalloc((void **)&c.guard_events, sizeof(int)));
    ORC_HIP(hipMemset(c.guard_events, 0, sizeof(int)));
    c.inited = true;
    return ORC_OK;
}

int orc_synchronize(void) {
    if (!orc::ctx().inited) return ORC_OK;
    ORC_HIP(hipStreamSynchronize(orc::ctx().stream));
    return ORC_OK;
}

const char *orc_last_error(void) { return orc::ctx().last_error.c_str(); }

int orc_device_memory(int64_t *free_bytes, int64_t *total_bytes) {
    ORC_TRY(orc::ensure_init());
    size_t f = 0, t = 0;
    ORC_HIP(hipMemGetInfo(&f, &t));
    if (free_bytes) *free_bytes = (int64_t)f;
    if (total_bytes) *total_bytes = (int64_t)t;
    return ORC_OK;
}

int orc_device_info(char *buf, int cap) {
    ORC_TRY(orc::ensure_init());
    if (!buf || cap <= 0) return orc::set_error(ORC_ERR_BAD_ARGUMENT, "null argument");
    hipDeviceProp_t prop;
    char bus[64] = "?";
    const int dev = orc::ctx().device;
    ORC_HIP(hipGetDeviceProperties(&prop, dev));
    (void)hipDeviceGetPCIBusId(bus, (int)sizeof(bus), dev);
    const int w = snprintf(buf, (size_t)cap, "%s | pci %s | ordinal %d | %d CUs", prop.name, bus, dev, prop.multiProcessorCount);
    if (w < 0 || w >= cap) return orc::set_error(ORC_ERR_BAD_ARGUMENT, "orc_device_info: buffer of %d bytes is too small", cap);
    return ORC_OK;
}

const char *orc_status_string(int st) {
    switch (st) {
    case ORC_OK: return "ok";
    case ORC_ERR_SOLUTION_DIVERGED: return "solution diverged";
    case ORC_ERR_MULTIGRID_DIVERGED: return "Multigrid diverged";
    case ORC_ERR_JACOBI_NAN: return "diverged";
    case ORC_ERR_JACOBI_TOO_LARGE: return "Diverged - max solution value > 10^10";
    case ORC_ERR_GS_MAINTENANCE: return "Gauss-Seidel out for maintenance :)";
    case ORC_ERR_STRUCTURAL_ZERO: return "Tried to access CsrMatrix element that hasn't been stored yet.";
    case ORC_ERR_UNSUPPORTED_BC: return "BC not supported";
    case ORC_ERR_UNSUPPORTED_SCHEME: return "unsupported scheme";
    case ORC_ERR_UNSUPPORTED_SOLVER: return "unsupported solution method";
    case ORC_ERR_BAD_ARGUMENT: return "bad argument";
    case ORC_ERR_NO_DEVICE: return "no HIP device (liborc_amd has no CPU fallback)";
    case ORC_ERR_HIP: return "HIP runtime error";
    case ORC_ERR_IO: return "I/O error";
    case ORC_ERR_COMM: return "RCCL error";
    case ORC_ERR_MESH_FORMAT: return "malformed mesh or data file";
    case ORC_ERR_NO_BOUNDARY_CONDITIONS: return "You must set boundary conditions.";
    case ORC_ERR_ZONE_NOT_FOUND: return "face zone should exist in mesh";
    case ORC_ERR_SINGULAR_MATRIX: return "called `Option::unwrap()` on a `None` value";
    default: return "unknown status";
    }
}

void orc_settings_default(OrcSettings *s) {
    memset(s, 0, sizeof(*s));
    s->momentum = ORC_MOMENTUM_CD1;
    s->diffusion = ORC_DIFFUSION_CD;
    s->pressure_interpolation = ORC_PINTERP_SECOND_ORDER;
    s->velocity_interpolation = ORC_VINTERP_RHIE_CHOW;
    s->gradient_reconstruction = ORC_GRAD_GREEN_GAUSS_CELL;
    s->pressure_relaxation = 0.01;
    s->momentum_relaxation = 0.5;
    s->solver_type = ORC_SOLVER_MULTIGRID;
    s->iterations = 50;
    s->relaxation = 0.5;
    s->relative_convergence_threshold = 1e-3;
    s->preconditioner = ORC_PRECOND_JACOBI;
    s->q1_compat = 1;
    s->breakdown_guard = 1;
    s->frozen_diagonals = 1;
    s->reduction_order = ORC_REDUCTION_TREE;
}

int orc_set_breakdown_guard(int on) {
    orc::ctx().breakdown_guard = on != 0;
    return ORC_OK;
}

int orc_set_reduction_order(int order) {
    if (order != ORC_REDUCTION_TREE && order != ORC_REDUCTION_REFERENCE) return orc::set_error(ORC_ERR_BAD_ARGUMENT, "unknown reduction order %d", order);
    orc::ctx().reduction_order = order;
    return ORC_OK;
}

int64_t orc_breakdown_guard_events(int reset) {
    orc::Ctx &c = orc::ctx();
    if (!c.inited || !c.guard_events) return 0;
    int h = 0;
    if (hipStreamSynchronize(c.stream) != hipSuccess) return -1;
    if (hipMemcpy(&h, c.guard_events, sizeof(int), hipMemcpyDeviceToHost) != hipSuccess) return -1;
    if (reset && hipMemset(c.guard_events, 0, sizeof(int)) != hipSuccess) return -1;
    return h;
}

long long orc_debug_halo_overlaps(void) { return orc::ctx().halo_overlaps; }
int orc_debug_clamp_partials_grid(long long requested) { return orc::clamp_partials_grid(requested); }
int orc_debug_max_partials(void) { return orc::kMaxPartials; }
int orc_debug_amg_certification(long long out[2], int reset) {
    if (!out) return orc::set_error(ORC_ERR_BAD_ARGUMENT, "null argument");
    orc::debug_amg_certification(out, reset != 0);
    return ORC_OK;
}
int orc_debug_amg_setup_stats(long long out[16], int reset) {
    if (!out) return orc::set_error(ORC_ERR_BAD_ARGUMENT, "null argument");
    orc::debug_amg_setup_stats(out, reset != 0);
    return ORC_OK;
}
long long orc_debug_shared_galerkin(int reset) { return orc::debug_shared_galerkin(reset != 0); }
int orc_debug_xwin_counters(long long out[3], int reset) {
    if (!out) return orc::set_error(ORC_ERR_BAD_ARGUMENT, "null argument");
    ORC_TRY(orc::ensure_init());
    return orc::debug_xwin_counters(out, reset != 0);
}

int orc_debug_product_launches(long long *out, int n_out, int reset) {
    if (n_out < 0 || (!out && n_out > 0)) { orc::set_error(ORC_ERR_BAD_ARGUMENT, "null argument"); return -1; }
    return orc::debug_product_launches(out, n_out, reset != 0);
}

int orc_debug_stream_report(char *buf, int cap) {
    if (!buf || cap <= 0) return -1;
    std::vector<orc::StreamEntry> copy;
    {
        std::lock_guard<std::mutex> lk(orc::g_streams_mu);
        copy = orc::g_streams;
    }
    int busy = 0, off = 0;
    for (const auto &e : copy) {
        const hipError_t q = hipStreamQuery(e.st);
        const char *state = q == hipSuccess ? "idle" : (q == hipErrorNotReady ? "busy" : hipGetErrorString(q));
        if (q == hipErrorNotReady) ++busy;
        const int w = snprintf(buf + off, (size_t)(cap - off), "%s priority %d %s\n", e.name.c_str(), e.priority, state);
        if (w < 0 || w >= cap - off) return -1;
        off += w;
    }
    return busy;
}

int orc_reload_environment(void) {
    orc::config_reload();
    return ORC_OK;
}

int orc_profile_enable(int on) {
    orc::ctx().profile = on != 0;
    return ORC_OK;
}

}
```

### orc_amd/csrc/spmv.hip

```cpp
#include <algorithm>
#include <atomic>
#include <cmath>
#include <cstdint>

#include "linalg_kernels.hpp"

namespace orc {

static inline int stream_nt(int64_t stream_bytes) {
    const int forced = cfg().spmv_nt;
    if (forced >= 0) return forced != 0;
    return stream_bytes > ((int64_t)128 << 20);
}

int matview_stream_nt(const MatView &A) { return stream_nt(A.pk.ptr && A.xw.lidx ? A.pk.total * 10 : A.P.padded * (A.P.col16 ? 10 : 12)); }

int spmv_grid(int32_t n_slices) {
    int64_t g = ((int64_t)n_slices + 3) / 4;
    const int cap = cfg().spmv_grid > 0 ? std::max(8, cfg().spmv_grid) : kMaxGrid;
    if (g > cap) g = cap;
    if (g >= 8) g = (g / 8) * 8;
    return clamp_partials_grid(g);
}

struct EpiStore {
    static constexpr int kReductions = 0;
    double *y;
    __device__ __forceinline__ void apply(int64_t row, double acc, double &, double &) const { y[row] = acc; }
};
struct EpiStoreSum {
    static constexpr int kReductions = 1;
    double *y;
    __device__ __forceinline__ void apply(int64_t row, double acc, double &r0, double &) const { y[row] = acc; r0 += acc; }
};
struct EpiResidual {
    static constexpr int kReductions = 1;
    const double *b;
    double *r, *p;
    __device__ __forceinline__ void apply(int64_t row, double acc, double &r0, double &) const {
        const double v = b[row] - acc;
        r[row] = v;
        if (p) p[row] = v;
        r0 += v;
    }
};
struct EpiResidualNorm {
    static constexpr int kReductions = 1;
    const double *b;
    double *r;
    __device__ __forceinline__ void apply(int64_t row, double acc, double &r0, double &) const {
        const double v = b[row] - acc;
        if (r) r[row] = v;
        r0 += v * v;
    }
};
struct EpiTs {
    static constexpr int kReductions = 2;
    const double *s;
    double *t;
    __device__ __forceinline__ void apply(int64_t row, double acc, double &r0, double &r1) const {
        t[row] = acc;
        r0 += acc * s[row];
        r1 += acc * acc;
    }
};
struct EpiStoreDot {
    static constexpr int kReductions = 1;
    const double *s;
    double *y;
    __device__ __forceinline__ void apply(int64_t row, double acc, double &r0, double &) const {
        y[row] = acc;
        r0 += acc * s[row];
    }
};

enum { kFamRagged = 0, kFamPacked, kFamWindow, kFamGenericScaled, kFamWide, kFamNarrow, kFamNarrowNT, kFamMesh, kFamCount };
static std::atomic<long long> g_product_launches[kFamCount];
static inline void count_launch(int family) { g_product_launches[family].fetch_add(1, std::memory_order_relaxed); }
int debug_product_launches(long long *out, int n_out, bool reset) {
    for (int f = 0; f < kFamCount; ++f) {
        const long long v = reset ? g_product_launches[f].exchange(0, std::memory_order_relaxed) : g_product_launches[f].load(std::memory_order_relaxed);
        if (out && f < n_out) out[f] = v;
    }
    for (int f = kFamCount; out && f < n_out; ++f) out[f] = 0;
    return kFamCount;
}

static int xwin_grid(MatView &A, int reductions) {
    const int per_cu = cfg().xwin_wgs_per_cu;
    static const int n_cu = [] {
        hipDeviceProp_t prop;
        int dev = 0;
        return (hipGetDevice(&dev) == hipSuccess && hipGetDeviceProperties(&prop, dev) == hipSuccess && prop.multiProcessorCount > 0) ? prop.multiProcessorCount : 256;
    }();
    int64_t gb = ((int64_t)A.P.n_slices + 3) / 4;
    const bool one_per_block = cfg().xwin_wg_per_block && (reductions == 0 || A.xw.fold_scratch != nullptr) && A.pk.total > 0;
    if (one_per_block) {
        const int64_t per_block = std::max<int64_t>(1, A.pk.total / std::max<int64_t>(gb, 1));
        const int64_t blocks_per_wg = std::min<int64_t>(4, std::max<int64_t>(1, (12000 + per_block / 2) / per_block));
        gb = (gb + blocks_per_wg - 1) / blocks_per_wg;
        gb = (gb + 7) / 8 * 8;
    } else {
        A.xw.fold_scratch = nullptr;
        if (gb > (int64_t)n_cu * per_cu) gb = (int64_t)n_cu * per_cu;
        gb = clamp_partials_grid(gb);
    }
    if (gb >= 8) gb = (gb / 8) * 8;
    return (int)std::max<int64_t>(gb, 1);
}

template <class View, class Exchange, class Launch>
static int launch_overlapped(const View &A, int g, int *grid_out, Exchange &&exchange, Launch &&launch) {
    HaloPlan *H = A.halo;
    const int g_b = std::max(8, (g / 8 / 8) * 8), g_i = std::max(8, ((g - 2 * g_b) / 8) * 8);
    const int total = g_i + 2 * g_b;
    if (grid_out) *grid_out = total;
    if (!H->aux_stream) {
        hipStream_t st2;
        hipEvent_t e1, e2;
        ORC_TRY(stream_create(&st2, kSolveStream, 0, "halo-overlap"));
        ORC_HIP(hipEventCreateWithFlags(&e1, hipEventDisableTiming));
        ORC_HIP(hipEventCreateWithFlags(&e2, hipEventDisableTiming));
        H->aux_stream = st2; H->ev_ready = e1; H->ev_done = e2;
    }
    hipStream_t lib = ctx().stream, aux = (hipStream_t)H->aux_stream;
    ORC_HIP(hipEventRecord((hipEvent_t)H->ev_ready, lib));
    ORC_HIP(hipStreamWaitEvent(aux, (hipEvent_t)H->ev_ready, 0));
    View V = A;
    V.part_stride = total;
    V.slice_lo = H->interior_lo; V.slice_hi = H->interior_hi; V.part_base = 0;
    const bool exchange_first = !comm_host_transport_active();
    if (exchange_first) ORC_TRY(exchange());
    launch(V, g_i, aux);
    ORC_HIP(hipEventRecord((hipEvent_t)H->ev_done, aux));
    if (!exchange_first) {
        const int ex = exchange();
        if (ex != ORC_OK) {
            (void)hipStreamWaitEvent(lib, (hipEvent_t)H->ev_done, 0);
            return ex;
        }
    }
    V.slice_lo = 0; V.slice_hi = H->interior_lo; V.part_base = g_i;
    launch(V, g_b, lib);
    V.slice_lo = H->interior_hi; V.slice_hi = A.P.n_slices; V.part_base = g_i + g_b;
    launch(V, g_b, lib);
    ORC_HIP(hipStreamWaitEvent(lib, (hipEvent_t)H->ev_done, 0));
    ORC_HIP(hipGetLastError());
    ctx().halo_overlaps += 1;
    return ORC_OK;
}
static inline bool overlap_pays(const HaloPlan *H, int32_t n_slices, int g) {
    return H && cfg().halo_overlap && ctx().world > 1 && g >= 64 && (int64_t)(H->interior_hi - H->interior_lo) * 2 >= (int64_t)n_slices;
}

template <class Epi, bool kMesh, bool kNarrow, bool kScaled, bool kNT>
static void launch_uniform_as(const MatView &A, int g, hipStream_t stream, const double *x, const Epi &epi, double *partials, const double *skip_flags) {
    static_assert(!(kScaled && kNT), "a scaled view is never streamed with the non-temporal hint");
    hipLaunchKernelGGL(HIP_KERNEL_NAME(spmv_uniform_k<Epi, false, kMesh, kNarrow, kScaled, kNT>), dim3(g), dim3(kBlock), 0, stream, A, x, epi, partials, skip_flags);
}
template <class Epi, bool kMesh, bool kNarrow>
static void launch_uniform(const MatView &A, int g, const double *x, const Epi &epi, double *partials, const double *skip_flags) {
    if (A.s1 || A.s2) launch_uniform_as<Epi, kMesh, kNarrow, true, false>(A, g, ctx().stream, x, epi, partials, skip_flags);
    else if (A.nt) launch_uniform_as<Epi, kMesh, kNarrow, false, true>(A, g, ctx().stream, x, epi, partials, skip_flags);
    else launch_uniform_as<Epi, kMesh, kNarrow, false, false>(A, g, ctx().stream, x, epi, partials, skip_flags);
}

template <class Epi>
static int launch_spmv(const MatView &A_in, const double *x, const Epi &epi, double *partials, int *grid_out, const double *skip_flags = nullptr) {
    MatView A = A_in;
    A.nt = matview_stream_nt(A);
    const bool xwin = A.xw.lidx != nullptr && A.pk.ptr != nullptr;
    const int g = xwin ? xwin_grid(A, Epi::kReductions) : spmv_grid(A.P.n_slices);
    const bool scaled = A.s1 || A.s2;
    const bool uniform_kernel = !A.pk.ptr && A.P.ragged != 1;
    if (uniform_kernel && A.slice_hi < 0 && overlap_pays(A.halo, A.P.n_slices, g))
        return launch_overlapped(A, g, grid_out, [&] { return A.halo->exchange(const_cast<double *>(x)); },
                                 [&](const MatView &V, int grid, hipStream_t stream) {
                                     launch_uniform_as<Epi, false, false, true, false>(V, grid, stream, x, epi, partials, skip_flags);
                                     count_launch(kFamGenericScaled);
                                 });
    if (grid_out) *grid_out = (xwin && Epi::kReductions > 0 && A.xw.fold_scratch) ? 1 : g;
    if (A.P.n == 0) return ORC_OK;
    if (A.halo) ORC_TRY(A.halo->exchange(const_cast<double *>(x)));
    if (xwin) {
        const size_t xwin_smem = sizeof(double) * (size_t)std::max(1, std::min(A.xw.cap, kXWinCap));
        if (!scaled && A.nt) hipLaunchKernelGGL(HIP_KERNEL_NAME(spmv_xwin_k<Epi, false, true>), dim3(g), dim3(kBlock), xwin_smem, ctx().stream, A, x, epi, partials, skip_flags);
        else if (!scaled) hipLaunchKernelGGL(HIP_KERNEL_NAME(spmv_xwin_k<Epi, false>), dim3(g), dim3(kBlock), xwin_smem, ctx().stream, A, x, epi, partials, skip_flags);
        else hipLaunchKernelGGL(HIP_KERNEL_NAME(spmv_xwin_k<Epi>), dim3(g), dim3(kBlock), xwin_smem, ctx().stream, A, x, epi, partials, skip_flags);
        count_launch(kFamWindow);
    } else if (A.pk.ptr) {
        hipLaunchKernelGGL(HIP_KERNEL_NAME(spmv_k<Epi, kSpmvPacked>), dim3(g), dim3(kBlock), 0, ctx().stream, A, x, epi, partials, skip_flags);
        count_launch(kFamPacked);
    } else if (A.P.ragged == 1) {
        hipLaunchKernelGGL(HIP_KERNEL_NAME(spmv_k<Epi, kSpmvRagged>), dim3(g), dim3(kBlock), 0, ctx().stream, A, x, epi, partials, skip_flags);
        count_launch(kFamRagged);
    } else if (A.persistent_pattern) {
        if (A.P.col16) launch_uniform<Epi, true, true>(A, g, x, epi, partials, skip_flags);
        else launch_uniform<Epi, true, false>(A, g, x, epi, partials, skip_flags);
        count_launch(kFamMesh);
    } else if (!scaled && A.P.col16) {
        if (A.nt) launch_uniform_as<Epi, false, true, false, true>(A, g, ctx().stream, x, epi, partials, skip_flags);
        else launch_uniform_as<Epi, false, true, false, false>(A, g, ctx().stream, x, epi, partials, skip_flags);
        count_launch(A.nt ? kFamNarrowNT : kFamNarrow);
    } else if (!scaled) {
        launch_uniform_as<Epi, false, false, false, false>(A, g, ctx().stream, x, epi, partials, skip_flags);
        count_launch(kFamWide);
    } else {
        launch_uniform_as<Epi, false, false, true, false>(A, g, ctx().stream, x, epi, partials, skip_flags);
        count_launch(kFamGenericScaled);
    }
    ORC_HIP(hipGetLastError());
    return ORC_OK;
}

int spmv_dev(const MatView &A, const double *x, double *y) { return launch_spmv(A, x, EpiStore{y}, nullptr, nullptr); }
int product_store(const MatView &A, const double *x, double *y, const double *skip_flags) {
    return launch_spmv(A, x, EpiStore{y}, nullptr, nullptr, skip_flags);
}
int product_store_sum(const MatView &A, const double *x, double *y, double *partials, int *grid_out, const double *skip_flags) {
    return launch_spmv(A, x, EpiStoreSum{y}, partials, grid_out, skip_flags);
}
int product_residual(const MatView &A, const double *x, const double *b, double *r, double *p, double *partials, int *grid_out, const double *skip_flags) {
    return launch_spmv(A, x, EpiResidual{b, r, p}, partials, grid_out, skip_flags);
}
int product_residual_norm(const MatView &A, const double *x, const double *b, double *r, double *partials, int *grid_out, const double *skip_flags) {
    return launch_spmv(A, x, EpiResidualNorm{b, r}, partials, grid_out, skip_flags);
}
int product_ts(const MatView &A, const double *s, double *t, double *partials, int *grid_out, const double *skip_flags) {
    return launch_spmv(A, s, EpiTs{s, t}, partials, grid_out, skip_flags);
}
int product_store_dot(const MatView &A, const double *p, double *q, double *partials, int *grid_out, const double *skip_flags) {
    return launch_spmv(A, p, EpiStoreDot{p, q}, partials, grid_out, skip_flags);
}

static double *unread_partials() {
    static double *const p = [] {
        double *q = nullptr;
        return hipMalloc((void **)&q, sizeof(double) * 3 * kMaxPartials) == hipSuccess ? q : nullptr;
    }();
    return p;
}
int residual_dev(const MatView &A, const double *b, const double *x, double *r) {
    int g = 0;
    double *dummy = unread_partials();
    if (!dummy) return set_error(ORC_ERR_HIP, "hipMalloc of the residual scratch failed");
    return launch_spmv(A, x, EpiResidual{b, r, nullptr}, dummy, &g);
}

int residual_norm2_dev(const MatView &A, const double *b, const double *x, double *partials, double *out, double *r_scratch) {
    int g = 0;
    const bool ref = reference_order(A) && r_scratch != nullptr;
    ORC_TRY(launch_spmv(A, x, EpiResidualNorm{b, ref ? r_scratch : nullptr}, partials, &g));
    if (ref) return dot_reference(r_scratch, r_scratch, A.P.n, out, nullptr);
    return reduce_partials(partials, g, 1, out, A.halo != nullptr);
}

__global__ __launch_bounds__(kBlock) void scale_values_k(MatView A, double *__restrict__ out) {
    const int lane = threadIdx.x & 63;
    SliceWalk w(A.P.n_slices);
    for (int64_t slice = w.begin; slice < w.end; slice += w.step) {
        const int64_t row = slice * 64 + lane;
        const int64_t base = A.P.slice_ptr[slice];
        const int width = (int)((A.P.slice_ptr[slice + 1] - base) >> 6);
        const bool live = row < A.P.n;
        const double s1 = (A.s1 && live) ? A.s1[row] : 1.;
        const double s2 = (A.s2 && live) ? A.s2[row] : 1.;
        for (int k = 0; k < width; ++k) {
            const int64_t p = base + (int64_t)k * 64 + lane;
            double t = A.val[p];
            if (A.s1) t = s1 * t;
            if (A.s2) t = s2 * t;
            out[p] = t;
        }
    }
}
static inline bool materialize_scaling(uint64_t iteration_count) {
    const int min_its = cfg().materialize_scaling;
    return min_its > 0 && iteration_count >= (uint64_t)min_its;
}

__global__ __launch_bounds__(kBlock) void scale_packed_k(MatView A, double *__restrict__ out) {
    const int lane = threadIdx.x & 63;
    SliceWalk w(A.P.n_slices);
    for (int64_t slice = w.begin; slice < w.end; slice += w.step) {
        const int64_t row = slice * 64 + lane;
        const int width = (int)((A.P.slice_ptr[slice + 1] - A.P.slice_ptr[slice]) >> 6);
        const bool live = row < A.P.n;
        const int len = live ? A.P.row_len[row] : 0;
        const double s1 = (A.s1 && live) ? A.s1[row] : 1.;
        const double s2 = (A.s2 && live) ? A.s2[row] : 1.;
        const f64x2_t *src = reinterpret_cast<const f64x2_t *>(A.pk.val + A.pk.ptr[slice]);
        f64x2_t *dst = reinterpret_cast<f64x2_t *>(out + A.pk.ptr[slice]);
        int off = 0;
        for (int k = 0; k < width; k += 2) {
            const bool in = k < len;
            const unsigned long long m = __ballot(in);
            const int rank = __builtin_amdgcn_mbcnt_hi((unsigned)(m >> 32), __builtin_amdgcn_mbcnt_lo((unsigned)m, 0u));
            if (in) {
                f64x2_t t = src[off + rank];
                if (A.s1) { t.x = s1 * t.x; t.y = s1 * t.y; }
                if (A.s2) { t.x = s2 * t.x; t.y = s2 * t.y; }
                dst[off + rank] = t;
            }
            off += __popcll(m);
        }
    }
}

int materialize_scaled_view(MatView &A, uint64_t iteration_count, Arena &arena) {
    if (!((A.s1 || A.s2) && A.P.n > 0 && materialize_scaling(iteration_count))) return ORC_OK;
    if (A.pk.ptr) {
        if (!(A.xw.lidx && A.pk.total > 0)) return ORC_OK;
        double *scaled;
        ORC_TRY(arena.alloc((size_t)A.pk.slots, &scaled));
        hipLaunchKernelGGL(scale_packed_k, dim3(spmv_grid(A.P.n_slices)), dim3(kBlock), 0, ctx().stream, A, scaled);
        ORC_HIP(hipGetLastError());
        A.pk.val = scaled;
        A.val = nullptr;
        A.s1 = A.s2 = nullptr;
        return ORC_OK;
    }
    if (A.P.padded <= 0) return ORC_OK;
    double *scaled;
    ORC_TRY(arena.alloc((size_t)A.P.padded, &scaled));
    hipLaunchKernelGGL(scale_values_k, dim3(spmv_grid(A.P.n_slices)), dim3(kBlock), 0, ctx().stream, A, scaled);
    ORC_HIP(hipGetLastError());
    A.val = scaled;
    A.s1 = A.s2 = nullptr;
    return ORC_OK;
}

template <class Fn>
static int time_launches(int reps, float *ms, Fn &&launch) {
    hipEvent_t e0, e1;
    ORC_HIP(hipEventCreate(&e0));
    ORC_HIP(hipEventCreate(&e1));
    int st = launch();
    if (st == ORC_OK && hipEventRecord(e0, ctx().stream) != hipSuccess) st = set_error(ORC_ERR_HIP, "hipEventRecord failed");
    for (int i = 0; i < reps && st == ORC_OK; ++i) st = launch();
    if (st == ORC_OK && (hipEventRecord(e1, ctx().stream) != hipSuccess || hipEventSynchronize(e1) != hipSuccess)) st = set_error(ORC_ERR_HIP, "hipEventRecord failed");
    if (st == ORC_OK && hipEventElapsedTime(ms, e0, e1) != hipSuccess) st = set_error(ORC_ERR_HIP, "hipEventElapsedTime failed");
    if (st == ORC_OK) *ms /= (float)std::max(reps, 1);
    (void)hipEventDestroy(e0);
    (void)hipEventDestroy(e1);
    return st;
}
int bench_inloop_products_dev(const MatView &A, const double *x, double *y, double *partials, int reps, float ms[2]) {
    int g = 0;
    ORC_TRY(time_launches(reps, &ms[0], [&] { return launch_spmv(A, x, EpiStoreSum{y}, partials, &g, nullptr); }));
    ORC_TRY(time_launches(reps, &ms[1], [&] { return launch_spmv(A, x, EpiTs{x, y}, partials, &g, nullptr); }));
    return ORC_OK;
}

struct EpiStore3 {
    static constexpr int kReductions = 0;
    double *y3;
    __device__ __forceinline__ void apply(int64_t row, const double (&acc)[3], double (&)[3][2]) const {
        reinterpret_cast<Vec3d *>(y3)[row] = Vec3d{acc[0], acc[1], acc[2]};
    }
};
struct EpiStoreSum3 {
    static constexpr int kReductions = 1;
    double *y3;
    __device__ __forceinline__ void apply(int64_t row, const double (&acc)[3], double (&red)[3][2]) const {
        reinterpret_cast<Vec3d *>(y3)[row] = Vec3d{acc[0], acc[1], acc[2]};
        red[0][0] += acc[0]; red[1][0] += acc[1]; red[2][0] += acc[2];
    }
};
struct EpiResidual3 {
    static constexpr int kReductions = 1;
    const double *b3;
    double *r3, *p3;
    __device__ __forceinline__ void apply(int64_t row, const double (&acc)[3], double (&red)[3][2]) const {
        const Vec3d b = reinterpret_cast<const Vec3d *>(b3)[row];
        const Vec3d v = {b.a - acc[0], b.b - acc[1], b.c - acc[2]};
        reinterpret_cast<Vec3d *>(r3)[row] = v;
        if (p3) reinterpret_cast<Vec3d *>(p3)[row] = v;
        red[0][0] += v.a; red[1][0] += v.b; red[2][0] += v.c;
    }
};
struct EpiResidualNorm3 {
    static constexpr int kReductions = 1;
    const double *b3;
    __device__ __forceinline__ void apply(int64_t row, const double (&acc)[3], double (&red)[3][2]) const {
        const Vec3d b = reinterpret_cast<const Vec3d *>(b3)[row];
        const double v0 = b.a - acc[0], v1 = b.b - acc[1], v2 = b.c - acc[2];
        red[0][0] += v0 * v0; red[1][0] += v1 * v1; red[2][0] += v2 * v2;
    }
};
struct EpiTs3 {
    static constexpr int kReductions = 2;
    const double *s3;
    double *t3;
    __device__ __forceinline__ void apply(int64_t row, const double (&acc)[3], double (&red)[3][2]) const {
        const Vec3d sv = reinterpret_cast<const Vec3d *>(s3)[row];
        reinterpret_cast<Vec3d *>(t3)[row] = Vec3d{acc[0], acc[1], acc[2]};
        red[0][0] += acc[0] * sv.a; red[0][1] += acc[0] * acc[0];
        red[1][0] += acc[1] * sv.b; red[1][1] += acc[1] * acc[1];
        red[2][0] += acc[2] * sv.c; red[2][1] += acc[2] * acc[2];
    }
};

template <class Epi3, bool kMesh, bool kNarrow, bool kScaled, bool kNT>
static void launch_uniform3_as(const MatView3 &A, int g, hipStream_t stream, const double *x3, const Epi3 &epi, double *partials) {
    static_assert(!(kScaled && kNT), "a scaled view is never streamed with the non-temporal hint");
    hipLaunchKernelGGL(HIP_KERNEL_NAME(spmv3_uniform_k<Epi3, 4, kMesh, kNarrow, kScaled, kNT>), dim3(g), dim3(kBlock), 0, stream, A, x3, epi, partials);
}
template <class Epi3, bool kMesh, bool kNarrow>
static void launch_uniform3(const MatView3 &A, int g, hipStream_t stream, const double *x3, const Epi3 &epi, double *partials) {
    if (A.s1 || A.s2) launch_uniform3_as<Epi3, kMesh, kNarrow, true, false>(A, g, stream, x3, epi, partials);
    else if (A.nt) launch_uniform3_as<Epi3, kMesh, kNarrow, false, true>(A, g, stream, x3, epi, partials);
    else launch_uniform3_as<Epi3, kMesh, kNarrow, false, false>(A, g, stream, x3, epi, partials);
}

template <class Epi3>
static int launch_spmv3(const MatView3 &A_in, const double *x3, const Epi3 &epi, double *partials, int *grid_out) {
    MatView3 A = A_in;
    A.nt = stream_nt(A.P.padded * (A.P.col16 ? 26 : 28));
    const int g = spmv_grid(A.P.n_slices);
    if (grid_out) *grid_out = g;
    if (A.P.n == 0) return ORC_OK;
    const bool scaled = A.s1 || A.s2;
    const bool plain_kernel = A.mesh_pattern && A.P.col16 != nullptr && !scaled;
    if (plain_kernel && overlap_pays(A.halo, A.P.n_slices, g))
        return launch_overlapped(A, g, grid_out, [&] { return A.halo->exchange_interleaved(const_cast<double *>(x3), 3); },
                                 [&](const MatView3 &V, int grid, hipStream_t stream) { launch_uniform3<Epi3, true, true>(V, grid, stream, x3, epi, partials); });
    if (A.halo) ORC_TRY(A.halo->exchange_interleaved(const_cast<double *>(x3), 3));
    hipStream_t stream = ctx().stream;
    if (A.mesh_pattern) {
        if (A.P.col16) launch_uniform3<Epi3, true, true>(A, g, stream, x3, epi, partials);
        else launch_uniform3<Epi3, true, false>(A, g, stream, x3, epi, partials);
    } else if (!scaled && A.P.col16 && A.nt) launch_uniform3_as<Epi3, false, true, false, true>(A, g, stream, x3, epi, partials);
    else if (!scaled && A.P.col16) launch_uniform3_as<Epi3, false, true, false, false>(A, g, stream, x3, epi, partials);
    else if (!scaled) launch_uniform3_as<Epi3, false, false, false, false>(A, g, stream, x3, epi, partials);
    else launch_uniform3_as<Epi3, false, false, true, false>(A, g, stream, x3, epi, partials);
    ORC_HIP(hipGetLastError());
    return ORC_OK;
}

int spmv3_dev(const MatView3 &A, const double *x3, double *y3) { return launch_spmv3(A, x3, EpiStore3{y3}, nullptr, nullptr); }
int product_store_sum3(const MatView3 &A, const double *x3, double *y3, double *partials, int *grid_out) {
    return launch_spmv3(A, x3, EpiStoreSum3{y3}, partials, grid_out);
}
int product_residual3(const MatView3 &A, const double *x3, const double *b3, double *r3, double *p3, double *partials, int *grid_out) {
    return launch_spmv3(A, x3, EpiResidual3{b3, r3, p3}, partials, grid_out);
}
int product_ts3(const MatView3 &A, const double *s3, double *t3, double *partials, int *grid_out) {
    return launch_spmv3(A, s3, EpiTs3{s3, t3}, partials, grid_out);
}

int residual3_dev(const MatView3 &A, const double *b3, double *x3, double *r3) {
    double *dummy = unread_partials();
    if (!dummy) return set_error(ORC_ERR_HIP, "hipMalloc of the residual scratch failed");
    return launch_spmv3(A, x3, EpiResidual3{b3, r3, nullptr}, dummy, nullptr);
}
int residual_norm2_3_dev(const MatView3 &A, const double *b3, double *x3, double *partials, double *out3) {
    int g = 0;
    ORC_TRY(launch_spmv3(A, x3, EpiResidualNorm3{b3}, partials, &g));
    return reduce_partials(partials, g, 3, out3, A.halo != nullptr);
}

__global__ __launch_bounds__(kBlock) void scale_values3_k(MatView3 A, int sys, double *__restrict__ out) {
    const int lane = threadIdx.x & 63;
    const double *__restrict__ val = A.val[sys];
    SliceWalk w(A.P.n_slices);
    for (int64_t slice = w.begin; slice < w.end; slice += w.step) {
        const int64_t row = slice * 64 + lane;
        const int64_t base = A.P.slice_ptr[slice];
        const int width = (int)((A.P.slice_ptr[slice + 1] - base) >> 6);
        const bool live = row < A.P.n;
        const double s1 = (A.s1 && live) ? A.s1[3 * row + sys] : 1.;
        const double s2 = (A.s2 && live) ? A.s2[3 * row + sys] : 1.;
        for (int k = 0; k < width; ++k) {
            const int64_t p = base + (int64_t)k * 64 + lane;
            double t = val[p];
            if (A.s1) t = s1 * t;
            if (A.s2) t = s2 * t;
            out[p] = t;
        }
    }
}

int materialize_scaled_view3(MatView3 &A, uint64_t iteration_count, Arena &arena) {
    if (!((A.s1 || A.s2) && A.P.padded > 0 && A.P.n > 0 && materialize_scaling(iteration_count))) return ORC_OK;
    for (int s = 0; s < 3; ++s) {
        double *scaled;
        ORC_TRY(arena.alloc((size_t)A.P.padded, &scaled));
        hipLaunchKernelGGL(scale_values3_k, dim3(spmv_grid(A.P.n_slices)), dim3(kBlock), 0, ctx().stream, A, s, scaled);
        A.val[s] = scaled;
    }
    ORC_HIP(hipGetLastError());
    A.s1 = A.s2 = nullptr;
    return ORC_OK;
}

int bench_inloop_products3_dev(const MatView3 &A, const double *x3, double *y3, double *partials, int reps, float ms[2]) {
    int g = 0;
    ORC_TRY(time_launches(reps, &ms[0], [&] { return launch_spmv3(A, x3, EpiStoreSum3{y3}, partials, &g); }));
    ORC_TRY(time_launches(reps, &ms[1], [&] { return launch_spmv3(A, x3, EpiTs3{x3, y3}, partials, &g); }));
    return ORC_OK;
}

}
```

### orc_amd/linear_algebra.py

```python
import ctypes as C

import numpy as np

from ._lib import check, lib


def _i64(a):
    return np.ascontiguousarray(a, dtype=np.int64)


def _f64(a):
    return np.ascontiguousarray(a, dtype=np.float64)


def _p(a, t):
    return a.ctypes.data_as(C.POINTER(t))


def iterative_solve(a, b, solution_vector, iteration_count, method, relaxation_factor, convergence_threshold,
                    preconditioner, raise_on_error=True):
    a = a.tocsr()
    a.sort_indices()
    rp, ci, v = _i64(a.indptr), _i64(a.indices), _f64(a.data)
    b = _f64(b)
    assert solution_vector.dtype == np.float64 and solution_vector.flags.c_contiguous
    st = lib().orc_iterative_solve(C.c_int64(a.shape[0]), _p(rp, C.c_int64), _p(ci, C.c_int64), _p(v, C.c_double),
                                   _p(b, C.c_double), _p(solution_vector, C.c_double), C.c_uint64(iteration_count),
                                   C.c_int(method), C.c_double(relaxation_factor), C.c_double(convergence_threshold),
                                   C.c_int(preconditioner))
    if raise_on_error:
        check(st)
    return st


def iterative_solve3(a_list, b_list, x_list, iteration_count, method, relaxation_factor, convergence_threshold, preconditioner):
    a0 = a_list[0]
    n = a0.shape[0]
    rp, ci = _i64(a0.indptr), _i64(a0.indices)
    for a in a_list[1:]:
        assert np.array_equal(a.indptr, a0.indptr) and np.array_equal(a.indices, a0.indices), "the three systems must share their pattern"
    vals = [_f64(a.data) for a in a_list]
    bs = [_f64(b) for b in b_list]
    for x in x_list:
        assert x.dtype == np.float64 and x.flags.c_contiguous and len(x) == n
    PD = C.POINTER(C.c_double)
    v3 = (PD * 3)(*[_p(v, C.c_double) for v in vals])
    b3 = (PD * 3)(*[_p(b, C.c_double) for b in bs])
    x3 = (PD * 3)(*[_p(x, C.c_double) for x in x_list])
    st3 = (C.c_int * 3)()
    st = lib().orc_iterative_solve3(C.c_int64(n), _p(rp, C.c_int64), _p(ci, C.c_int64), v3, b3, x3, C.c_uint64(iteration_count), C.c_int(method),
                                    C.c_double(relaxation_factor), C.c_double(convergence_threshold), C.c_int(preconditioner), st3)
    return st, [st3[0], st3[1], st3[2]]


def set_breakdown_guard(on):
    check(lib().orc_set_breakdown_guard(C.c_int(1 if on else 0)))


def set_reduction_order(order):
    check(lib().orc_set_reduction_order(C.c_int(int(order))))


def breakdown_guard_events(reset=False):
    lib().orc_breakdown_guard_events.restype = C.c_int64
    return int(lib().orc_breakdown_guard_events(C.c_int(1 if reset else 0)))


def last_jacobi_sweeps():
    return lib().orc_last_jacobi_sweeps()


def set_gmres_restart(m):
    check(lib().orc_set_gmres_restart(C.c_int(int(m))))


def last_gmres_stats():
    steps, cycles = C.c_int64(0), C.c_int64(0)
    beta0, est = C.c_double(0.0), C.c_double(0.0)
    check(lib().orc_last_gmres_stats(C.byref(steps), C.byref(cycles), C.byref(beta0), C.byref(est)))
    return steps.value, cycles.value, beta0.value, est.value


def last_cg_stats():
    its, ev = C.c_int64(0), C.c_int32(0)
    beta0, res = C.c_double(0.0), C.c_double(0.0)
    check(lib().orc_last_cg_stats(C.byref(its), C.byref(beta0), C.byref(res), C.byref(ev)))
    return its.value, beta0.value, res.value, ev.value


def csr_spmv(a, x, reps=1):
    a = a.tocsr()
    a.sort_indices()
    rp, ci, v = _i64(a.indptr), _i64(a.indices), _f64(a.data)
    x = _f64(x)
    y = np.empty(a.shape[0])
    ms = C.c_double(0.0)
    check(lib().orc_csr_spmv(C.c_int64(a.shape[0]), _p(rp, C.c_int64), _p(ci, C.c_int64), _p(v, C.c_double),
                             _p(x, C.c_double), _p(y, C.c_double), C.c_int(reps), C.byref(ms)))
    return y, ms.value


def amg_coarsen(a):
    import scipy.sparse as sp
    a = a.tocsr()
    a.sort_indices()
    n = a.shape[0]
    rp, ci, v = _i64(a.indptr), _i64(a.indices), _f64(a.data)
    partner = np.empty(n, np.int64)
    nc, nnz, rounds = C.c_int64(0), C.c_int64(0), C.c_int(0)
    args = (C.c_int64(n), _p(rp, C.c_int64), _p(ci, C.c_int64), _p(v, C.c_double), _p(partner, C.c_int64), C.byref(nc), C.byref(nnz))
    check(lib().orc_amg_coarsen(*args, None, None, None, C.byref(rounds)))
    orp, oci, ov = np.empty(nc.value + 1, np.int64), np.empty(nnz.value, np.int64), np.empty(nnz.value)
    check(lib().orc_amg_coarsen(*args, _p(orp, C.c_int64), _p(oci, C.c_int64), _p(ov, C.c_double), C.byref(rounds)))
    return partner, sp.csr_matrix((ov, oci, orp), shape=(nc.value, nc.value)), rounds.value


def debug_coloring(a):
    a = a.tocsr()
    a.sort_indices()
    n = a.shape[0]
    rp, ci = _i64(a.indptr), _i64(a.indices)
    colors = np.empty(n, np.int32)
    nc = C.c_int32(0)
    check(lib().orc_debug_coloring(C.c_int64(n), _p(rp, C.c_int64), _p(ci, C.c_int64), _p(colors, C.c_int32), C.byref(nc)))
    return colors, nc.value


def amg_coarse_product(a, x, scaled=False):
    a = a.tocsr()
    a.sort_indices()
    n = a.shape[0]
    rp, ci, v = _i64(a.indptr), _i64(a.indices), _f64(a.data)
    x = _f64(x)
    assert len(x) == (n + 1) // 2
    y = np.empty(len(x))
    mirror = C.c_int(0)
    check(lib().orc_debug_amg_coarse_product(C.c_int64(n), _p(rp, C.c_int64), _p(ci, C.c_int64), _p(v, C.c_double), C.c_int(1 if scaled else 0),
                                             _p(x, C.c_double), _p(y, C.c_double), C.byref(mirror)))
    return y, bool(mirror.value)


def amg_packed_mirror(a):
    a = a.tocsr()
    a.sort_indices()
    n = a.shape[0]
    rp, ci, v = _i64(a.indptr), _i64(a.indices), _f64(a.data)
    sizes = np.zeros(5, np.int64)
    f = lib().orc_debug_amg_packed_mirror
    null = [None] * 8
    check(f(C.c_int64(n), _p(rp, C.c_int64), _p(ci, C.c_int64), _p(v, C.c_double), _p(sizes, C.c_int64), *null))
    nc, ns, slots, pos_slots, nb = (int(t) for t in sizes)
    if slots == 0:
        return None
    out = dict(row_len=np.empty(nc, np.int32), pk_ptr=np.empty(ns + 1, np.int64), pk_col=np.empty(slots, np.int32), pk_val=np.empty(slots),
               lptr=np.empty(ns + 1, np.int64), lidx=np.empty(pos_slots, np.uint16), wcol=np.empty((nb, 5000), np.int32), wsize=np.empty(nb, np.int32))
    check(f(C.c_int64(n), _p(rp, C.c_int64), _p(ci, C.c_int64), _p(v, C.c_double), _p(sizes, C.c_int64), _p(out["row_len"], C.c_int32),
            _p(out["pk_ptr"], C.c_int64), _p(out["pk_col"], C.c_int32), _p(out["pk_val"], C.c_double), _p(out["lptr"], C.c_int64),
            _p(out["lidx"], C.c_uint16), _p(out["wcol"], C.c_int32), _p(out["wsize"], C.c_int32)))
    return out


def xwin_counters(reset=False):
    out = (C.c_longlong * 3)()
    check(lib().orc_debug_xwin_counters(out, C.c_int(1 if reset else 0)))
    return out[0], out[1], out[2]


def shared_galerkin(reset=False):
    f = lib().orc_debug_shared_galerkin
    f.restype = C.c_longlong
    return int(f(C.c_int(1 if reset else 0)))


def amg_certification(reset=False):
    out = (C.c_longlong * 2)()
    check(lib().orc_debug_amg_certification(out, C.c_int(1 if reset else 0)))
    return out[0], out[1]


AMG_SETUP_FIELDS = ("list", "steps", "scans", "longest", "overflow", "changed", "fallback_sweeps", "lanes")


def amg_setup_stats(reset=False):
    out = (C.c_longlong * 16)()
    check(lib().orc_debug_amg_setup_stats(out, C.c_int(1 if reset else 0)))
    d = dict(zip(AMG_SETUP_FIELDS, (int(v) for v in out[:8])))
    d["fallback"] = 1 if d["fallback_sweeps"] > 0 else 0
    d["tiers"] = [int(v) for v in out[8:15]]
    d["max_cand"] = int(out[15])
    return d


PRODUCT_FAMILIES = ("ragged", "packed", "window", "generic_scaled", "wide", "narrow", "narrow_nt", "mesh")


def product_launches(reset=False):
    out = (C.c_longlong * len(PRODUCT_FAMILIES))()
    n = lib().orc_debug_product_launches(out, C.c_int(len(PRODUCT_FAMILIES)), C.c_int(1 if reset else 0))
    if n != len(PRODUCT_FAMILIES):
        raise RuntimeError("orc_debug_product_launches: %d families, %d expected" % (n, len(PRODUCT_FAMILIES)))
    return dict(zip(PRODUCT_FAMILIES, (int(v) for v in out)))
```

Before: 1.418.

## Compact AMG window SpMV indices to 12-bit positions and 16-bit segment columns

Adds a compact encoding for the AMG coarse-level window SpMV. Local positions are packed as 12-bit values (three words per eight slots instead of four), and window column lists are stored as per-64-entry segment bases plus 16-bit offsets whenever they fit. The SpMV kernel gains a template variant that decodes both formats, cutting index bandwidth in this memory-bound product at the cost of extra bit manipulation and a build-time fit check. The new path is on by default through ORC_XWIN_COMPACT, and debug hooks are added to inspect the raw packed data.

```diff
diff --git a/include/orc_amd.h b/include/orc_amd.h
--- a/include/orc_amd.h
+++ b/include/orc_amd.h
@@ -204,6 +204,8 @@
                                  double *y, int *has_window_mirror);
 int orc_debug_amg_packed_mirror(int64_t n, const int64_t *row_ptr, const int64_t *col_idx, const double *values, int64_t sizes[5], int32_t *row_len,
                                 int64_t *pk_ptr, int32_t *pk_col, double *pk_val, int64_t *lptr, uint16_t *lidx, int32_t *wcol, int32_t *wsize);
+int orc_debug_amg_xwin_raw(int64_t n, const int64_t *row_ptr, const int64_t *col_idx, const double *values, int64_t info[10], int64_t *lptr,
+                           unsigned char *pos_raw, int32_t *wcol_raw, int32_t *wsize, int32_t *wfmt);
 long long orc_debug_collectives(int reset);
 int orc_debug_clamp_partials_grid(long long requested);
 int orc_debug_max_partials(void);
diff --git a/orc_amd/csrc/amg_hooks.hip b/orc_amd/csrc/amg_hooks.hip
--- a/orc_amd/csrc/amg_hooks.hip
+++ b/orc_amd/csrc/amg_hooks.hip
@@ -1,4 +1,5 @@
 #include <algorithm>
+#include <cstring>
 
 #include "amg.hpp"
 
@@ -62,6 +63,24 @@
     return ORC_OK;
 }
 
+static void expand_positions12(const unsigned *raw, int64_t n_slots, uint16_t *out) {
+    for (int64_t g = 0; g < n_slots / kPackChunk; ++g) {
+        const unsigned long long lo = raw[3 * g] | (unsigned long long)raw[3 * g + 1] << 32, hi = raw[3 * g + 1] >> 16 | (unsigned long long)raw[3 * g + 2] << 16;
+        for (int u = 0; u < 4; ++u) {
+            out[kPackChunk * g + u] = (uint16_t)(lo >> (12 * u) & 0xfffu);
+            out[kPackChunk * g + 4 + u] = (uint16_t)(hi >> (12 * u) & 0xfffu);
+        }
+    }
+}
+static void expand_window16(int32_t *words, int ws) {
+    const int nseg = (ws + kXWinSeg - 1) / kXWinSeg;
+    const std::vector<int32_t> base(words, words + nseg);
+    std::vector<uint16_t> off((size_t)ws);
+    memcpy(off.data(), words + nseg, sizeof(uint16_t) * (size_t)ws);
+    for (int j = 0; j < ws; ++j) words[j] = base[(size_t)(j / kXWinSeg)] + (int32_t)off[(size_t)j];
+}
+static size_t position_bytes(const XWinDev &xw, int64_t n_slots) { return (size_t)n_slots * (xw.pos12 ? 3 : 4) / 2; }
+
 int amg_debug_packed(const MatView &A, Arena &arena, int64_t sizes[5], int32_t *row_len_h, int64_t *pk_ptr_h, int32_t *pk_col_h, double *pk_val_h,
                      int64_t *lptr_h, uint16_t *lidx_h, int32_t *wcol_h, int32_t *wsize_h) {
     hipStream_t st = ctx().stream;
@@ -79,10 +98,50 @@
         ORC_HIP(hipMemcpyAsync(pk_col_h, L.pk.col, sizeof(int32_t) * (size_t)sizes[2], hipMemcpyDeviceToHost, st));
         ORC_HIP(hipMemcpyAsync(pk_val_h, L.pk.val, sizeof(double) * (size_t)sizes[2], hipMemcpyDeviceToHost, st));
         ORC_HIP(hipMemcpyAsync(lptr_h, L.xw.lptr, sizeof(int64_t) * (size_t)(ns + 1), hipMemcpyDeviceToHost, st));
-        ORC_HIP(hipMemcpyAsync(lidx_h, L.xw.lidx, sizeof(uint16_t) * (size_t)sizes[3], hipMemcpyDeviceToHost, st));
+        std::vector<unsigned> raw(L.xw.pos12 ? position_bytes(L.xw, sizes[3]) / 4 : 0);
+        std::vector<int32_t> wfmt((size_t)nb);
+        if (L.xw.pos12) ORC_HIP(hipMemcpyAsync(raw.data(), L.xw.lidx, position_bytes(L.xw, sizes[3]), hipMemcpyDeviceToHost, st));
+        else ORC_HIP(hipMemcpyAsync(lidx_h, L.xw.lidx, sizeof(uint16_t) * (size_t)sizes[3], hipMemcpyDeviceToHost, st));
         ORC_HIP(hipMemcpyAsync(wcol_h, L.xw.wcol, sizeof(int32_t) * (size_t)(nb * kXWinCap), hipMemcpyDeviceToHost, st));
         ORC_HIP(hipMemcpyAsync(wsize_h, L.xw.wsize, sizeof(int32_t) * (size_t)nb, hipMemcpyDeviceToHost, st));
+        ORC_HIP(hipMemcpyAsync(wfmt.data(), L.xw.wfmt, sizeof(int32_t) * (size_t)nb, hipMemcpyDeviceToHost, st));
         ORC_HIP(hipStreamSynchronize(st));
+        if (L.xw.pos12) expand_positions12(raw.data(), sizes[3], lidx_h);
+        for (int64_t b = 0; b < nb; ++b)
+            if (wfmt[(size_t)b] && wsize_h[b] > 0) expand_window16(wcol_h + b * kXWinCap, wsize_h[b]);
+    }
+    return ORC_OK;
+}
+
+int amg_debug_xwin_raw(const MatView &A, Arena &arena, int64_t info[10], int64_t *lptr_h, unsigned char *pos_raw_h, int32_t *wcol_raw_h, int32_t *wsize_h, int32_t *wfmt_h) {
+    hipStream_t st = ctx().stream;
+    ArenaScope scope(arena);
+    AmgHierarchy::Level L;
+    ORC_TRY(build_level(A, arena, L));
+    const bool mirror = L.pk.ptr && L.xw.lidx;
+    const int64_t ns = L.P.n_slices, nb = (ns + 3) / 4;
+    for (int i = 0; i < 10; ++i) info[i] = 0;
+    info[0] = L.n; info[1] = ns;
+    if (!mirror) return ORC_OK;
+    std::vector<int32_t> wsize((size_t)nb), wfmt((size_t)nb);
+    ORC_HIP(hipMemcpyAsync(&info[3], L.xw.lptr + ns, sizeof(int64_t), hipMemcpyDeviceToHost, st));
+    ORC_HIP(hipMemcpyAsync(wsize.data(), L.xw.wsize, sizeof(int32_t) * (size_t)nb, hipMemcpyDeviceToHost, st));
+    ORC_HIP(hipMemcpyAsync(wfmt.data(), L.xw.wfmt, sizeof(int32_t) * (size_t)nb, hipMemcpyDeviceToHost, st));
+    ORC_HIP(hipStreamSynchronize(st));
+    info[2] = nb; info[4] = L.xw.pos12 ? 12 : 16; info[5] = (int64_t)position_bytes(L.xw, info[3]); info[6] = L.xw.cap;
+    for (int64_t b = 0; b < nb; ++b) {
+        const int64_t ws = wsize[(size_t)b];
+        if (ws <= 0) continue;
+        if (wfmt[(size_t)b]) { ++info[7]; info[9] += 2 * ws + 4 * ((ws + kXWinSeg - 1) / kXWinSeg); }
+        else { ++info[8]; info[9] += 4 * ws; }
+    }
+    if (lptr_h && pos_raw_h && wcol_raw_h && wsize_h && wfmt_h) {
+        ORC_HIP(hipMemcpyAsync(lptr_h, L.xw.lptr, sizeof(int64_t) * (size_t)(ns + 1), hipMemcpyDeviceToHost, st));
+        ORC_HIP(hipMemcpyAsync(pos_raw_h, L.xw.lidx, (size_t)info[5], hipMemcpyDeviceToHost, st));
+        ORC_HIP(hipMemcpyAsync(wcol_raw_h, L.xw.wcol, sizeof(int32_t) * (size_t)(nb * kXWinCap), hipMemcpyDeviceToHost, st));
+        ORC_HIP(hipStreamSynchronize(st));
+        std::copy(wsize.begin(), wsize.end(), wsize_h);
+        std::copy(wfmt.begin(), wfmt.end(), wfmt_h);
     }
     return ORC_OK;
 }
diff --git a/orc_amd/csrc/amg_mirror.hip b/orc_amd/csrc/amg_mirror.hip
--- a/orc_amd/csrc/amg_mirror.hip
+++ b/orc_amd/csrc/amg_mirror.hip
@@ -1,4 +1,6 @@
 #include <algorithm>
+#include <mutex>
+#include <vector>
 
 #include "amg.hpp"
 
@@ -7,23 +9,28 @@
 constexpr int kXBitWords = 8192;
 __device__ unsigned long long g_xwin_counters[3];
 constexpr int kXBitWordsSmall = 4096;
+constexpr int kXFmtPos12 = 1, kXFmtCol16 = 2, kXFmtRedo = 4;
+constexpr int kXWinSegs = (kXWinCap + kXWinSeg - 1) / kXWinSeg;
 template <int kWords, bool kSecond>
-__global__ __launch_bounds__(kBlock) void xwin_build_k(SellDev P, const int64_t *__restrict__ lptr, int *__restrict__ wcol, int *__restrict__ wsize,
+__global__ __launch_bounds__(kBlock) void xwin_build_k(SellDev P, const int64_t *__restrict__ lptr, int *__restrict__ wcol, int *__restrict__ wsize, int *__restrict__ wfmt,
                                                        unsigned short *__restrict__ lidx, int64_t n_blocks, int win_cap, int bit_words, int pass_words,
-                                                       int *__restrict__ pending ) {
+                                                       int *__restrict__ pending , int fmt) {
     if (kSecond && *pending == 0) return;
     __shared__ unsigned bits[kWords];
     __shared__ unsigned short wpre[kWords];
     __shared__ int s_min, s_max, s_part[kBlock];
+    __shared__ int s_segbase[kXWinSegs], s_wide;
+    const bool redo = (fmt & kXFmtRedo) != 0;
     const int tid = threadIdx.x, lane = tid & 63, wave = tid >> 6;
     unsigned long long n_built = 0, n_capped = 0, n_spanned = 0;
     for (int64_t b = blockIdx.x; b < n_blocks; b += gridDim.x) {
         if (kSecond && wsize[b] != -2) continue;
+        if (redo && wsize[b] <= 0) continue;
         const int64_t row = b * kXWinRows + tid;
         const bool live = row < P.n;
         const int len = live ? P.row_len[row] : 0;
         const int64_t rbase = live ? P.slice_ptr[row >> 6] + (row & 63) : 0;
-        if (tid == 0) { s_min = 0x7fffffff; s_max = -1; }
+        if (tid == 0) { s_min = 0x7fffffff; s_max = -1; s_wide = 0; }
         __syncthreads();
         if (len > 0) {
             atomicMin(&s_min, P.col[rbase]);
@@ -37,12 +44,12 @@
             __syncthreads();
             continue;
         }
-        if (!kSecond && words <= bit_words && words > pass_words) {
+        if (!kSecond && !redo && words <= bit_words && words > pass_words) {
             if (tid == 0) { wsize[b] = -2; atomicAdd(pending, 1); }
             __syncthreads();
             continue;
         }
-        ++n_built;
+        if (!redo) ++n_built;
         if (words > bit_words || words > kWords) {
             if (tid == 0) wsize[b] = -1;
             ++n_spanned;
@@ -77,16 +84,59 @@
         }
         int run = s_part[tid] - local;
         int *wc = wcol + b * kXWinCap;
-        for (int w = tid * per; w < words && w < (tid + 1) * per; ++w) {
-            wpre[w] = (unsigned short)run;
-            unsigned m = bits[w];
-            while (m) {
-                const int bit = __ffs(m) - 1;
-                wc[run++] = cmin + (w << 5) + bit;
-                m &= m - 1;
-            }
-        }
-        if (tid == 0) wsize[b] = total;
+        bool col16 = false;
+        if ((fmt & kXFmtCol16) && !redo) {
+            int r = run;
+            for (int w = tid * per; w < words && w < (tid + 1) * per; ++w) {
+                unsigned m = bits[w];
+                while (m) {
+                    if ((r & (kXWinSeg - 1)) == 0) s_segbase[r / kXWinSeg] = cmin + (w << 5) + (__ffs(m) - 1);
+                    ++r;
+                    m &= m - 1;
+                }
+            }
+            __syncthreads();
+            bool wide = false;
+            r = run;
+            for (int w = tid * per; w < words && w < (tid + 1) * per; ++w) {
+                unsigned m = bits[w];
+                while (m) {
+                    wide |= cmin + (w << 5) + (__ffs(m) - 1) - s_segbase[r / kXWinSeg] > 65535;
+                    ++r;
+                    m &= m - 1;
+                }
+            }
+            if (wide) s_wide = 1;
+            __syncthreads();
+            col16 = s_wide == 0;
+        }
+        if (col16) {
+            const int nseg = (total + kXWinSeg - 1) / kXWinSeg;
+            unsigned short *w16 = reinterpret_cast<unsigned short *>(wc + nseg);
+            for (int w = tid * per; w < words && w < (tid + 1) * per; ++w) {
+                wpre[w] = (unsigned short)run;
+                unsigned m = bits[w];
+                while (m) {
+                    const int bit = __ffs(m) - 1;
+                    w16[run] = (unsigned short)(cmin + (w << 5) + bit - s_segbase[run / kXWinSeg]);
+                    ++run;
+                    m &= m - 1;
+                }
+            }
+            for (int sg = tid; sg < nseg; sg += kBlock) wc[sg] = s_segbase[sg];
+        } else {
+            for (int w = tid * per; w < words && w < (tid + 1) * per; ++w) {
+                wpre[w] = (unsigned short)run;
+                unsigned m = bits[w];
+                while (m) {
+                    const int bit = __ffs(m) - 1;
+                    if (!redo) wc[run] = cmin + (w << 5) + bit;
+                    ++run;
+                    m &= m - 1;
+                }
+            }
+        }
+        if (tid == 0 && !redo) { wsize[b] = total; wfmt[b] = col16 ? 1 : 0; }
         __syncthreads();
         const int64_t slice = b * 4 + wave;
         if (slice < P.n_slices) {
@@ -98,23 +148,31 @@
                 const unsigned long long m = __ballot(in);
                 const int rank = __builtin_amdgcn_mbcnt_hi((unsigned)(m >> 32), __builtin_amdgcn_mbcnt_lo((unsigned)m, 0u));
                 if (in) {
-                    u32x4_t w = {0u, 0u, 0u, 0u};
+                    unsigned pos[kPackChunk];
 #pragma unroll
                     for (int u = 0; u < kPackChunk; ++u) {
+                        pos[u] = 0u;
                         if (j0 + u < len) {
                             const int c = P.col[sbase + (int64_t)(j0 + u) * 64 + lane] - cmin;
-                            const unsigned pos = wpre[c >> 5] + __popc(bits[c >> 5] & ((1u << (c & 31)) - 1u));
-                            w[u >> 1] |= pos << (16 * (u & 1));
+                            pos[u] = wpre[c >> 5] + __popc(bits[c >> 5] & ((1u << (c & 31)) - 1u));
                         }
                     }
-                    *reinterpret_cast<u32x4_t *>(lidx + off + (int64_t)kPackChunk * rank) = w;
+                    if (fmt & kXFmtPos12) {
+#pragma unroll
+                        for (int u = 0; u < kPackChunk; ++u) pos[u] &= 0xfffu;
+                        const u32x3_t w = {pos[0] | pos[1] << 12 | pos[2] << 24, pos[2] >> 8 | pos[3] << 4 | pos[4] << 16 | pos[5] << 28, pos[5] >> 4 | pos[6] << 8 | pos[7] << 20};
+                        *reinterpret_cast<u32x3_a4_t *>(reinterpret_cast<unsigned *>(lidx) + ((off >> 3) + rank) * 3) = w;
+                    } else {
+                        const u32x4_t w = {pos[0] | pos[1] << 16, pos[2] | pos[3] << 16, pos[4] | pos[5] << 16, pos[6] | pos[7] << 16};
+                        *reinterpret_cast<u32x4_t *>(lidx + off + (int64_t)kPackChunk * rank) = w;
+                    }
                 }
                 off += (int64_t)kPackChunk * __popcll(m);
             }
         }
         __syncthreads();
     }
-    if (tid == 0) {
+    if (tid == 0 && !redo) {
         if (n_built) atomicAdd(&g_xwin_counters[0], n_built);
         if (n_capped) atomicAdd(&g_xwin_counters[1], n_capped);
         if (n_spanned) atomicAdd(&g_xwin_counters[2], n_spanned);
@@ -136,12 +194,22 @@
         if (c[q]) atomicAdd(over + q, c[q]);
 }
 
-__global__ __launch_bounds__(kBlock) void xwin_stats_k(const int *__restrict__ wcol, const int *__restrict__ wsize, int64_t n_blocks, unsigned long long *__restrict__ out) {
+struct XWinList {
+    const int *wc;
+    int fmt, nseg;
+    __device__ int operator[](int j) const { return fmt ? wc[j / kXWinSeg] + (int)reinterpret_cast<const unsigned short *>(wc + nseg)[j] : wc[j]; }
+};
+__global__ __launch_bounds__(kBlock) void xwin_stats_k(const int *__restrict__ wcol, const int *__restrict__ wsize, const int *__restrict__ wfmt, int64_t n_blocks,
+                                                       unsigned long long *__restrict__ out) {
+    __shared__ int s_wide;
     for (int64_t b = blockIdx.x; b < n_blocks; b += gridDim.x) {
         const int ws = wsize[b];
         if (ws <= 0) { if (threadIdx.x == 0 && ws < 0) atomicAdd(out + 4, 1ull); continue; }
-        const int *wc = wcol + b * kXWinCap;
+        const XWinList wc{wcol + b * kXWinCap, wfmt[b], (ws + kXWinSeg - 1) / kXWinSeg};
+        if (threadIdx.x == 0) s_wide = 0;
+        __syncthreads();
         unsigned long long runs = 0, long_entries = 0;
+        bool wide = false;
         for (int j = threadIdx.x; j < ws; j += kBlock) {
             if (j == 0 || wc[j] != wc[j - 1] + 1) {
                 ++runs;
@@ -149,13 +217,18 @@
                 while (e < ws && wc[e] == wc[e - 1] + 1) ++e;
                 if (e - j >= 8) long_entries += (unsigned long long)(e - j);
             }
-        }
+            wide |= wc[j] - wc[j & ~(kXWinSeg - 1)] > 65535;
+        }
+        if (wide) s_wide = 1;
         atomicAdd(out + 1, runs);
         atomicAdd(out + 2, long_entries);
+        __syncthreads();
         if (threadIdx.x == 0) {
             atomicAdd(out + 0, (unsigned long long)ws);
             if (wc[ws - 1] - wc[0] < 65536) atomicAdd(out + 3, 1ull);
-        }
+            if (!s_wide) { atomicAdd(out + 5, 1ull); atomicAdd(out + 6, (unsigned long long)ws); }
+        }
+        __syncthreads();
     }
 }
 
@@ -216,6 +289,23 @@
     return ORC_OK;
 }
 
+static std::mutex g_large_share_mu;
+static std::vector<int64_t> g_large_share_rows;
+static bool large_share_expected(int64_t nc) {
+    std::lock_guard<std::mutex> lk(g_large_share_mu);
+    return std::find(g_large_share_rows.begin(), g_large_share_rows.end(), nc) != g_large_share_rows.end();
+}
+static void expect_large_share(int64_t nc, bool large) {
+    std::lock_guard<std::mutex> lk(g_large_share_mu);
+    const auto it = std::find(g_large_share_rows.begin(), g_large_share_rows.end(), nc);
+    if (large && it == g_large_share_rows.end()) {
+        if (g_large_share_rows.size() >= 64) g_large_share_rows.erase(g_large_share_rows.begin());
+        g_large_share_rows.push_back(nc);
+    } else if (!large && it != g_large_share_rows.end()) {
+        g_large_share_rows.erase(it);
+    }
+}
+
 int build_windows(const GalerkinSibling *sys, int n_sys, const int64_t *lptr, int64_t pos_slots, Arena &tmp) {
     AmgHierarchy::Level &L = *sys[0].L;
     Arena &arena = *sys[0].arena;
@@ -224,22 +314,31 @@
     hipStream_t st = ctx().stream;
     const bool trace = cfg().amg_trace;
     const int64_t n_blocks = ((int64_t)Pc.n_slices + 3) / 4;
-    int *wcol, *wsize;
+    int *wcol, *wsize, *wfmt;
     unsigned short *lidx;
     ORC_TRY(arena.alloc((size_t)n_blocks * kXWinCap, &wcol));
     ORC_TRY(arena.alloc((size_t)n_blocks, &wsize));
-    ORC_TRY(arena.alloc((size_t)std::max<int64_t>(pos_slots, 1), &lidx));
+    ORC_TRY(arena.alloc((size_t)n_blocks, &wfmt));
+    ORC_HIP(hipMemsetAsync(wfmt, 0, sizeof(int) * (size_t)n_blocks, st));
     const int win_cap = cfg().xwin_cap > 0 ? std::min(kXWinCap, cfg().xwin_cap) : kXWinCap;
     const int bit_words = cfg().xwin_bitwords > 0 ? std::min(kXBitWords, cfg().xwin_bitwords) : kXBitWords;
     const int small_words = cfg().xwin_small_bitwords > 0 ? std::min(kXBitWordsSmall, cfg().xwin_small_bitwords) : kXBitWordsSmall;
-    int *pending;
+    int *pending, *over;
     ORC_TRY(tmp.alloc((size_t)1, &pending));
+    ORC_TRY(tmp.alloc((size_t)kXWinCapSizes, &over));
     ORC_HIP(hipMemsetAsync(pending, 0, sizeof(int), st));
-    hipLaunchKernelGGL(HIP_KERNEL_NAME(xwin_build_k<kXBitWordsSmall, false>), dim3((unsigned)std::min<int64_t>(n_blocks, 2048)), dim3(kBlock), 0, st, Pc, lptr, wcol, wsize, lidx,
-                       n_blocks, win_cap, bit_words, small_words, pending);
+    const bool compact = cfg().xwin_compact;
+    const bool share_known = win_cap <= kXWinPos12Max || !cfg().xwin_level_cap;
+    const bool pos12_first = compact && (share_known ? win_cap <= kXWinPos12Max : !large_share_expected(nc));
+    const int fmt = (pos12_first ? kXFmtPos12 : 0) | (compact ? kXFmtCol16 : 0);
+    const size_t pos_units = (size_t)std::max<int64_t>(pos_slots, 1);
+    const Arena::Mark before_positions = arena.mark();
+    ORC_TRY(arena.alloc(pos12_first ? pos_units / 4 * 3 + 2 : pos_units, &lidx));
+    hipLaunchKernelGGL(HIP_KERNEL_NAME(xwin_build_k<kXBitWordsSmall, false>), dim3((unsigned)std::min<int64_t>(n_blocks, 2048)), dim3(kBlock), 0, st, Pc, lptr, wcol, wsize, wfmt, lidx,
+                       n_blocks, win_cap, bit_words, small_words, pending, fmt);
     if (bit_words > small_words)
-        hipLaunchKernelGGL(HIP_KERNEL_NAME(xwin_build_k<kXBitWords, true>), dim3((unsigned)std::min<int64_t>(n_blocks, 2048)), dim3(kBlock), 0, st, Pc, lptr, wcol, wsize, lidx,
-                           n_blocks, win_cap, bit_words, kXBitWords, pending);
+        hipLaunchKernelGGL(HIP_KERNEL_NAME(xwin_build_k<kXBitWords, true>), dim3((unsigned)std::min<int64_t>(n_blocks, 2048)), dim3(kBlock), 0, st, Pc, lptr, wcol, wsize, wfmt, lidx,
+                           n_blocks, win_cap, bit_words, kXBitWords, pending, fmt);
     if (trace) {
         int hp = 0;
         ORC_HIP(hipMemcpyAsync(&hp, pending, sizeof(int), hipMemcpyDeviceToHost, st));
@@ -247,9 +346,7 @@
         fprintf(stderr, "[amg windows n=%lld] %lld blocks, %d left to the full bitmap\n", (long long)nc, (long long)n_blocks, hp);
     }
     ORC_HIP(hipGetLastError());
-    L.xw.wcol = wcol; L.xw.wsize = wsize; L.xw.lidx = lidx; L.xw.lptr = lptr;
-    int *over;
-    ORC_TRY(tmp.alloc((size_t)kXWinCapSizes, &over));
+    L.xw.wcol = wcol; L.xw.wsize = wsize; L.xw.wfmt = wfmt; L.xw.lidx = lidx; L.xw.lptr = lptr;
     ORC_HIP(hipMemsetAsync(over, 0, kXWinCapSizes * sizeof(int), st));
     hipLaunchKernelGGL(xwin_cap_k, dim3((unsigned)std::max<int64_t>(1, std::min<int64_t>((n_blocks + kBlock - 1) / kBlock, 64))), dim3(kBlock), 0, st, (const int *)wsize, n_blocks, over);
     int h_over[kXWinCapSizes];
@@ -259,6 +356,17 @@
     for (int q = 0; q < kXWinCapSizes && cfg().xwin_level_cap; ++q)
         if (kXWinCapSize[q] <= win_cap && (int64_t)h_over[q] * 100 <= n_blocks) { cap = kXWinCapSize[q]; break; }
     L.xw.cap = cap;
+    L.xw.pos12 = compact && cap <= kXWinPos12Max ? 1 : 0;
+    if (compact && !share_known) expect_large_share(nc, !L.xw.pos12);
+    if ((L.xw.pos12 != 0) != pos12_first) {
+        arena.release(before_positions);
+        ORC_TRY(arena.alloc(L.xw.pos12 ? pos_units / 4 * 3 + 2 : pos_units, &lidx));
+        hipLaunchKernelGGL(HIP_KERNEL_NAME(xwin_build_k<kXBitWords, false>), dim3((unsigned)std::min<int64_t>(n_blocks, 2048)), dim3(kBlock), 0, st, Pc, lptr, wcol, wsize, wfmt, lidx,
+                           n_blocks, win_cap, bit_words, kXBitWords, pending, kXFmtRedo | (L.xw.pos12 ? kXFmtPos12 : 0));
+        ORC_HIP(hipGetLastError());
+        L.xw.lidx = lidx;
+        if (trace) fprintf(stderr, "[amg windows n=%lld] LDS share %d entries: positions rewritten in %d bits\n", (long long)nc, cap, L.xw.pos12 ? 12 : 16);
+    }
     if (trace) fprintf(stderr, "[amg windows n=%lld] LDS share %d entries per workgroup (%d of %lld blocks have larger windows)\n", (long long)nc, cap,
                        cap < win_cap ? h_over[std::find(kXWinCapSize, kXWinCapSize + kXWinCapSizes, cap) - kXWinCapSize] : 0, (long long)n_blocks);
     for (int s = 0; s < n_sys; ++s) {
@@ -273,15 +381,16 @@
         xw.fold_scratch = fs; xw.fold_counter = fc;
     }
     if (cfg().debug_xwin) {
-        unsigned long long *d_st, h_st[5];
-        ORC_TRY(tmp.alloc((size_t)5, &d_st));
+        unsigned long long *d_st, h_st[7];
+        ORC_TRY(tmp.alloc((size_t)7, &d_st));
         ORC_HIP(hipMemsetAsync(d_st, 0, sizeof(h_st), st));
-        hipLaunchKernelGGL(xwin_stats_k, dim3((unsigned)std::min<int64_t>(n_blocks, 4096)), dim3(kBlock), 0, st, (const int *)wcol, (const int *)wsize, n_blocks, d_st);
+        hipLaunchKernelGGL(xwin_stats_k, dim3((unsigned)std::min<int64_t>(n_blocks, 4096)), dim3(kBlock), 0, st, (const int *)wcol, (const int *)wsize, (const int *)wfmt, n_blocks, d_st);
         ORC_HIP(hipMemcpyAsync(h_st, d_st, sizeof(h_st), hipMemcpyDeviceToHost, st));
         ORC_HIP(hipStreamSynchronize(st));
-        fprintf(stderr, "[orc xwin] rows %lld nnz %lld blocks %lld: window entries %llu (%.1f per row), runs %llu (%.1f entries per run), in runs >= 8: %.1f %%, span < 65536: %llu blocks, no window: %llu\n",
+        fprintf(stderr, "[orc xwin] rows %lld nnz %lld blocks %lld: window entries %llu (%.1f per row), runs %llu (%.1f entries per run), in runs >= 8: %.1f %%, span < 65536: %llu blocks, no window: %llu; every 64-entry segment < 65536: %llu blocks with %llu window entries (%.2f %%); positions %d bits\n",
                 (long long)nc, (long long)L.pk.total, (long long)n_blocks, h_st[0], (double)h_st[0] / (double)nc, h_st[1], (double)h_st[0] / (double)std::max<unsigned long long>(h_st[1], 1),
-                100. * (double)h_st[2] / (double)std::max<unsigned long long>(h_st[0], 1), h_st[3], h_st[4]);
+                100. * (double)h_st[2] / (double)std::max<unsigned long long>(h_st[0], 1), h_st[3], h_st[4], h_st[5], h_st[6],
+                100. * (double)h_st[6] / (double)std::max<unsigned long long>(h_st[0], 1), L.xw.pos12 ? 12 : 16);
     }
     return ORC_OK;
 }
diff --git a/orc_amd/csrc/api_linalg.cpp b/orc_amd/csrc/api_linalg.cpp
--- a/orc_amd/csrc/api_linalg.cpp
+++ b/orc_amd/csrc/api_linalg.cpp
@@ -206,6 +206,17 @@
     return amg_debug_packed(m.view, arena, sizes, row_len, pk_ptr, pk_col, pk_val, lptr, lidx, wcol, wsize);
 }
 
+int orc_debug_amg_xwin_raw(int64_t n, const int64_t *row_ptr, const int64_t *col_idx, const double *values, int64_t info[10], int64_t *lptr,
+                           unsigned char *pos_raw, int32_t *wcol_raw, int32_t *wsize, int32_t *wfmt) {
+    using namespace orc;
+    ORC_TRY(ensure_init());
+    if (n < 1 || !row_ptr || !col_idx || !values || !info) return set_error(ORC_ERR_BAD_ARGUMENT, "null argument");
+    UserMatrix m;
+    ORC_TRY(m.load(n, row_ptr, col_idx, values));
+    Arena arena;
+    return amg_debug_xwin_raw(m.view, arena, info, lptr, pos_raw, wcol_raw, wsize, wfmt);
+}
+
 int orc_debug_coloring(int64_t n, const int64_t *row_ptr, const int64_t *col_idx, int32_t *colors, int32_t *n_colors) {
     using namespace orc;
     ORC_TRY(ensure_init());
diff --git a/orc_amd/csrc/arms.hpp b/orc_amd/csrc/arms.hpp
--- a/orc_amd/csrc/arms.hpp
+++ b/orc_amd/csrc/arms.hpp
@@ -40,6 +40,8 @@
                       int scaled = 0, int *mirror_out = nullptr);
 int amg_debug_packed(const MatView &A, Arena &arena, int64_t sizes[5], int32_t *row_len_h, int64_t *pk_ptr_h, int32_t *pk_col_h, double *pk_val_h,
                      int64_t *lptr_h, uint16_t *lidx_h, int32_t *wcol_h, int32_t *wsize_h);
+int amg_debug_xwin_raw(const MatView &A, Arena &arena, int64_t info[10], int64_t *lptr_h, unsigned char *pos_raw_h, int32_t *wcol_raw_h, int32_t *wsize_h,
+                       int32_t *wfmt_h);
 void gs_forget_pattern(const void *col_ptr);
 int bench_gs_sweep_dev(const MatView &A, const double *b, double *x, int reps, Arena &arena, float *ms_per_sweep, int *n_colors);
 int bench_gs_sweep0_dev(const MatView A[3], const double *const b[3], int reps, Arena &arena, float ms[2], int *n_colors);
diff --git a/orc_amd/csrc/config.hpp b/orc_amd/csrc/config.hpp
--- a/orc_amd/csrc/config.hpp
+++ b/orc_amd/csrc/config.hpp
@@ -29,6 +29,7 @@
     int xwin_small_bitwords = 0;
     bool xwin_wg_per_block = true;
     bool xwin_level_cap = true;
+    bool xwin_compact = true;
     bool gs_slotspace = true;
     bool trace = false;
     bool amg_trace = false;
diff --git a/orc_amd/csrc/linalg.hpp b/orc_amd/csrc/linalg.hpp
--- a/orc_amd/csrc/linalg.hpp
+++ b/orc_amd/csrc/linalg.hpp
@@ -37,11 +37,15 @@
 
 constexpr int kXWinRows = 256;
 constexpr int kXWinCap = 5000;
+constexpr int kXWinPos12Max = 4096;
+constexpr int kXWinSeg = 64;
 struct XWinDev {
     const int32_t *wcol = nullptr;
     const int32_t *wsize = nullptr;
+    const int32_t *wfmt = nullptr;
     const uint16_t *lidx = nullptr;
     const int64_t *lptr = nullptr;
+    int32_t pos12 = 0;
     int32_t cap = kXWinCap;
     double *fold_scratch = nullptr;
     unsigned *fold_counter = nullptr;
diff --git a/orc_amd/csrc/linalg_kernels.hpp b/orc_amd/csrc/linalg_kernels.hpp
--- a/orc_amd/csrc/linalg_kernels.hpp
+++ b/orc_amd/csrc/linalg_kernels.hpp
@@ -19,6 +19,13 @@
 typedef unsigned u32x4_t __attribute__((ext_vector_type(4)));
 typedef int i32x2_t __attribute__((ext_vector_type(2)));
 typedef double f64x2_t __attribute__((ext_vector_type(2)));
+typedef unsigned u32x3_t __attribute__((ext_vector_type(3)));
+typedef u32x3_t u32x3_a4_t __attribute__((aligned(4)));
+template <bool NT>
+__device__ __forceinline__ u32x3_t ld_pos12(const unsigned *p) {
+    if (NT) return __builtin_nontemporal_load(reinterpret_cast<const u32x3_a4_t *>(p));
+    return *reinterpret_cast<const u32x3_a4_t *>(p);
+}
 
 __device__ __forceinline__ int packed_pair(bool in, int &off) {
     const unsigned long long m = __ballot(in);
@@ -326,7 +333,7 @@
     }
 }
 
-template <class Epi, bool kScaled = true, bool kNT = false>
+template <class Epi, bool kScaled = true, bool kNT = false, bool kP12 = false>
 __global__ __launch_bounds__(kBlock) void spmv_xwin_k(MatView A, const double *__restrict__ x, Epi epi, double *__restrict__ partials,
                                                       const double *__restrict__ skip_flags) {
     __shared__ double lds[8];
@@ -365,6 +372,7 @@
         const int64_t sb = __builtin_amdgcn_readfirstlane((int)(pk_off & 0xffffffff)) | ((int64_t)__builtin_amdgcn_readfirstlane((int)(pk_off >> 32)) << 32);
         const int64_t lb = __builtin_amdgcn_readfirstlane((int)(lp_off & 0xffffffff)) | ((int64_t)__builtin_amdgcn_readfirstlane((int)(lp_off >> 32)) << 32);
         const u32x4_t *s_pos = reinterpret_cast<const u32x4_t *>(A.xw.lidx + lb);
+        const unsigned *s_pos12 = reinterpret_cast<const unsigned *>(A.xw.lidx) + (lb >> 3) * 3;
         const f64x2_t *s_val = reinterpret_cast<const f64x2_t *>(A.pk.val + sb);
         int poff = 0, voff = 0;
         u32x4_t c, cn;
@@ -373,13 +381,40 @@
             {
                 const unsigned long long m = __ballot(k0 < len);
                 const int rank = __builtin_amdgcn_mbcnt_hi((unsigned)(m >> 32), __builtin_amdgcn_mbcnt_lo((unsigned)m, 0u));
-                cc = ld_stream<kNT>(s_pos + poff + (k0 < len ? rank : 0));
+                const int slot = poff + (k0 < len ? rank : 0);
+                if (kP12) {
+                    const u32x3_t w = ld_pos12<kNT>(s_pos12 + 3 * slot);
+                    cc = u32x4_t{w.x, w.y, w.z, 0u};
+                } else {
+                    cc = ld_stream<kNT>(s_pos + slot);
+                }
                 poff += __popcll(m);
             }
 #pragma unroll
             for (int q = 0; q < kC / 2; ++q) vv[q] = ld_stream<kNT>(s_val + packed_pair(k0 + 2 * q < len, voff));
         };
-        if (ws > 0) {
+        if (ws > 0 && A.xw.wfmt[b]) {
+            const int nseg = (ws + kXWinSeg - 1) / kXWinSeg;
+            const int32_t *wb = A.xw.wcol + b * kXWinCap;
+            const uint16_t *w16 = reinterpret_cast<const uint16_t *>(wb + nseg);
+            for (int j0 = 0; j0 < ws; j0 += 8 * kBlock) {
+                int wj[8];
+                double xw[8];
+#pragma unroll
+                for (int q = 0; q < 8; ++q) {
+                    const int j = j0 + q * kBlock + (int)threadIdx.x;
+                    const int seg = min((j0 + q * kBlock + wave * 64) / kXWinSeg, nseg - 1);
+                    wj[q] = wb[seg] + (int)ld_stream<kNT>(w16 + (j < ws ? j : ws - 1));
+                }
+#pragma unroll
+                for (int q = 0; q < 8; ++q) xw[q] = x[wj[q]];
+#pragma unroll
+                for (int q = 0; q < 8; ++q) {
+                    const int j = j0 + q * kBlock + (int)threadIdx.x;
+                    if (j < ws) xs[j] = xw[q];
+                }
+            }
+        } else if (ws > 0) {
             const int32_t *wc = A.xw.wcol + b * kXWinCap;
             for (int j0 = 0; j0 < ws; j0 += 8 * kBlock) {
                 int wj[8];
@@ -406,11 +441,18 @@
             if (ws >= 0) {
                 auto consume = [&](int k0, const u32x4_t &cc, const f64x2_t (&vv)[kC / 2]) {
                     double xv[kC];
-#pragma unroll
-                    for (int q = 0; q < kC / 2; ++q) {
-                        const unsigned w = cc[q];
-                        xv[2 * q] = xs[w & 0xffffu];
-                        xv[2 * q + 1] = xs[w >> 16];
+                    if (kP12) {
+                        const unsigned w0 = cc[0], w1 = cc[1], w2 = cc[2];
+                        const unsigned o[kC] = {w0 << 3, w0 >> 9, __builtin_amdgcn_alignbit(w1, w0, 21), w1 >> 1, w1 >> 13, __builtin_amdgcn_alignbit(w2, w1, 25), w2 >> 5, w2 >> 17};
+#pragma unroll
+                        for (int u = 0; u < kC; ++u) xv[u] = *reinterpret_cast<const double *>(reinterpret_cast<const char *>(xs) + (o[u] & 0x7ff8u));
+                    } else {
+#pragma unroll
+                        for (int q = 0; q < kC / 2; ++q) {
+                            const unsigned w = cc[q];
+                            xv[2 * q] = xs[w & 0xffffu];
+                            xv[2 * q + 1] = xs[w >> 16];
+                        }
                     }
 #pragma unroll
                     for (int u = 0; u < kC; ++u) {
diff --git a/orc_amd/csrc/runtime.cpp b/orc_amd/csrc/runtime.cpp
--- a/orc_amd/csrc/runtime.cpp
+++ b/orc_amd/csrc/runtime.cpp
@@ -63,6 +63,7 @@
     c.xwin_small_bitwords = env_int("ORC_XWIN_SMALL_BITWORDS", 0);
     c.xwin_wg_per_block = env_on("ORC_XWIN_WG_PER_BLOCK", true);
     c.xwin_level_cap = env_on("ORC_XWIN_LEVEL_CAP", true);
+    c.xwin_compact = env_on("ORC_XWIN_COMPACT", true);
     c.gs_slotspace = env_on("ORC_GS_SLOTSPACE", true);
     c.trace = env_set("ORC_DEBUG_TRACE");
     c.amg_trace = env_set("ORC_AMG_TRACE");
diff --git a/orc_amd/csrc/spmv.hip b/orc_amd/csrc/spmv.hip
--- a/orc_amd/csrc/spmv.hip
+++ b/orc_amd/csrc/spmv.hip
@@ -163,6 +163,13 @@
     if (A.s1 || A.s2) launch_uniform_as<Epi, kMesh, kNarrow, true, false>(A, g, ctx().stream, x, epi, partials, skip_flags);
     else if (A.nt) launch_uniform_as<Epi, kMesh, kNarrow, false, true>(A, g, ctx().stream, x, epi, partials, skip_flags);
     else launch_uniform_as<Epi, kMesh, kNarrow, false, false>(A, g, ctx().stream, x, epi, partials, skip_flags);
+}
+
+template <class Epi, bool kP12>
+static void launch_xwin(const MatView &A, int g, size_t smem, bool scaled, const double *x, const Epi &epi, double *partials, const double *skip_flags) {
+    if (!scaled && A.nt) hipLaunchKernelGGL(HIP_KERNEL_NAME(spmv_xwin_k<Epi, false, true, kP12>), dim3(g), dim3(kBlock), smem, ctx().stream, A, x, epi, partials, skip_flags);
+    else if (!scaled) hipLaunchKernelGGL(HIP_KERNEL_NAME(spmv_xwin_k<Epi, false, false, kP12>), dim3(g), dim3(kBlock), smem, ctx().stream, A, x, epi, partials, skip_flags);
+    else hipLaunchKernelGGL(HIP_KERNEL_NAME(spmv_xwin_k<Epi, true, false, kP12>), dim3(g), dim3(kBlock), smem, ctx().stream, A, x, epi, partials, skip_flags);
 }
 
 template <class Epi>
@@ -184,9 +191,8 @@
     if (A.halo) ORC_TRY(A.halo->exchange(const_cast<double *>(x)));
     if (xwin) {
         const size_t xwin_smem = sizeof(double) * (size_t)std::max(1, std::min(A.xw.cap, kXWinCap));
-        if (!scaled && A.nt) hipLaunchKernelGGL(HIP_KERNEL_NAME(spmv_xwin_k<Epi, false, true>), dim3(g), dim3(kBlock), xwin_smem, ctx().stream, A, x, epi, partials, skip_flags);
-        else if (!scaled) hipLaunchKernelGGL(HIP_KERNEL_NAME(spmv_xwin_k<Epi, false>), dim3(g), dim3(kBlock), xwin_smem, ctx().stream, A, x, epi, partials, skip_flags);
-        else hipLaunchKernelGGL(HIP_KERNEL_NAME(spmv_xwin_k<Epi>), dim3(g), dim3(kBlock), xwin_smem, ctx().stream, A, x, epi, partials, skip_flags);
+        if (A.xw.pos12) launch_xwin<Epi, true>(A, g, xwin_smem, scaled, x, epi, partials, skip_flags);
+        else launch_xwin<Epi, false>(A, g, xwin_smem, scaled, x, epi, partials, skip_flags);
         count_launch(kFamWindow);
     } else if (A.pk.ptr) {
         hipLaunchKernelGGL(HIP_KERNEL_NAME(spmv_k<Epi, kSpmvPacked>), dim3(g), dim3(kBlock), 0, ctx().stream, A, x, epi, partials, skip_flags);
diff --git a/orc_amd/linear_algebra.py b/orc_amd/linear_algebra.py
--- a/orc_amd/linear_algebra.py
+++ b/orc_amd/linear_algebra.py
@@ -160,6 +160,53 @@
     return out
 
 
+def xwin_unpack_positions(raw, bits):
+    raw = np.ascontiguousarray(raw, np.uint8)
+    if bits == 16:
+        return raw.view(np.uint16).copy()
+    assert bits == 12 and len(raw) % 12 == 0
+    w = raw.view(np.uint32).reshape(-1, 3).astype(np.uint64)
+    lo = w[:, 0] | (w[:, 1] << np.uint64(32))
+    hi = (w[:, 1] >> np.uint64(16)) | (w[:, 2] << np.uint64(16))
+    out = np.empty((len(w), 8), np.uint16)
+    for u in range(4):
+        out[:, u] = (lo >> np.uint64(12 * u)) & np.uint64(0xfff)
+        out[:, 4 + u] = (hi >> np.uint64(12 * u)) & np.uint64(0xfff)
+    return out.reshape(-1)
+
+
+def xwin_unpack_window(words, wsize, fmt):
+    words = np.ascontiguousarray(words, np.int32)
+    if wsize <= 0:
+        return np.empty(0, np.int32)
+    if not fmt:
+        return words[:wsize].copy()
+    nseg = (wsize + 63) // 64
+    off = words[nseg:nseg + (wsize + 1) // 2].view(np.uint16)[:wsize].astype(np.int32)
+    return words[:nseg][np.arange(wsize) // 64] + off
+
+
+def amg_xwin_raw(a):
+    a = a.tocsr()
+    a.sort_indices()
+    n = a.shape[0]
+    rp, ci, v = _i64(a.indptr), _i64(a.indices), _f64(a.data)
+    info = np.zeros(10, np.int64)
+    f = lib().orc_debug_amg_xwin_raw
+    head = (C.c_int64(n), _p(rp, C.c_int64), _p(ci, C.c_int64), _p(v, C.c_double), _p(info, C.c_int64))
+    check(f(*head, None, None, None, None, None))
+    nc, ns, nb, pos_slots, bits, pos_bytes = (int(t) for t in info[:6])
+    if nb == 0:
+        return None
+    out = dict(lptr=np.empty(ns + 1, np.int64), pos_raw=np.empty(pos_bytes, np.uint8), wcol_raw=np.empty((nb, 5000), np.int32),
+               wsize=np.empty(nb, np.int32), wfmt=np.empty(nb, np.int32))
+    check(f(*head, _p(out["lptr"], C.c_int64), _p(out["pos_raw"], C.c_uint8), _p(out["wcol_raw"], C.c_int32), _p(out["wsize"], C.c_int32),
+            _p(out["wfmt"], C.c_int32)))
+    out.update(pos_bits=int(info[4]), pos_bytes=int(info[5]), cap=int(info[6]), blocks_col16=int(info[7]), blocks_col32=int(info[8]),
+               wcol_bytes=int(info[9]), pos_slots=pos_slots)
+    return out
+
+
 def xwin_counters(reset=False):
     out = (C.c_longlong * 3)()
     check(lib().orc_debug_xwin_counters(out, C.c_int(1 if reset else 0)))
```

Measured after the change: 1.441 (median of 6 runs). 1.02x the previous value.
